# Boese0601/RC-MVSNet

Hardware: AMD Instinct MI355X
Metric: ref-scenes/sec (DTU 3-view 512x640, D=48/32/8) (higher is better)
Workload: dtype f32; 1 GPU; BASELINE configs[1]: CascadeMVSNet_eval.forward, DTU-shaped 3 views 512x640, D=(48,32,8), batch 1 per GPU, fp32, random-init seeded weights; views=3, height=512, width=640, parallelism=scene-per-gpu x1, ranks=1, procs_per_gpu=1, rccl_ranks=0

## Files before the change

rc_mvsnet_amd/_lib.py:

```python
import ast
import ctypes
import os
import re
import subprocess

_HERE = os.path.dirname(os.path.abspath(__file__))
LIB_PATH = os.path.join(_HERE, "librcmvs_hip.so")
CSRC = os.path.join(_HERE, "csrc")
HEADER = os.path.join(os.path.dirname(_HERE), "include", "rcmvs.h")

_lib = None


class RcmvsError(RuntimeError):
    pass


_CTYPES = {"int": ctypes.c_int, "float": ctypes.c_float, "double": ctypes.c_double, "long long": ctypes.c_longlong}


def _const_expr(text):
    def ev(node):
        if isinstance(node, ast.Constant) and type(node.value) is int:
            return node.value
        if isinstance(node, ast.BinOp) and isinstance(node.op, ast.LShift):
            return ev(node.left) << ev(node.right)
        raise ValueError(text)
    return ev(ast.parse(text.strip(), mode="eval").body)


def _ctype(decl, what, c_type):
    if c_type not in _CTYPES:
        raise RcmvsError(f"{HEADER}: `{decl}`: {what} type `{c_type}` is outside the ABI's types ({', '.join(_CTYPES)}, pointers)")
    return _CTYPES[c_type]


def parse_header(text):
    text = re.sub(r"/\*.*?\*/|//[^\n]*", " ", text, flags=re.S)
    signatures, restypes, constants, code = {}, {}, {}, []
    for line in text.splitlines():
        if not line.lstrip().startswith("#"):
            code.append(line)
            continue
        m = re.match(r"\s*#\s*define\s+(RCMVS_\w+)\s+(\S.*)", line)
        if m:
            try:
                value = _const_expr(m.group(2))
            except (ValueError, SyntaxError):
                raise RcmvsError(f"{HEADER}: `{line.strip()}`: not an integer expression of literals, << and parentheses") from None
            if m.group(1) in constants:
                raise RcmvsError(f"{HEADER}: {m.group(1)} is defined twice")
            constants[m.group(1)] = value
    for decl in re.sub(r'extern\s+"C"\s*\{', " ", "\n".join(code)).split(";"):
        decl = " ".join(decl.split())
        if "rcmvs_" not in decl:
            continue
        m = re.fullmatch(r"([\w\s*]+?)\s*\b(rcmvs_\w+)\s*\(([^()]*)\)", decl)
        if not m:
            raise RcmvsError(f"{HEADER}: `{decl}` is not a complete `<type> rcmvs_name(<parameters>);` declaration")
        ret, name, params = m.group(1), m.group(2), m.group(3).strip()
        if name in signatures:
            raise RcmvsError(f"{HEADER}: {name} is declared twice")
        if ret.replace("const", "").replace(" ", "") == "char*":
            restypes[name] = ctypes.c_char_p
        elif ret != "int":
            restypes[name] = _ctype(decl, "return", ret)
        argtypes = []
        for param in ([] if params == "void" else params.split(",")):
            if "*" in param:
                argtypes.append(ctypes.c_void_p)
                continue
            words = [w for w in param.split() if w != "const"]
            if len(words) < 2 or not words[-1].isidentifier():
                raise RcmvsError(f"{HEADER}: `{decl}`: parameter `{param.strip()}` is not `<type> <name>`")
            argtypes.append(_ctype(decl, "parameter", " ".join(words[:-1])))
        signatures[name] = argtypes
    return signatures, restypes, constants


def _read_header():
    try:
        with open(HEADER) as f:
            return f.read()
    except FileNotFoundError:
        raise RcmvsError(f"{HEADER} is missing: the ctypes binding is derived from the C header, which was expected there "
                         "(include/rcmvs.h next to the rc_mvsnet_amd package)") from None


SIGNATURES, _RESTYPES, CONSTANTS = parse_header(_read_header())
REQUIRED_VERSION = CONSTANTS["RCMVS_VERSION"]


def sources():
    return sorted(os.path.join(CSRC, f) for f in os.listdir(CSRC) if f.endswith(".hip"))


def build(force=False, verbose=False):
    from concurrent.futures import ThreadPoolExecutor
    srcs = sources()
    hdrs = [os.path.join(CSRC, f) for f in os.listdir(CSRC) if f.endswith(".h")] + [HEADER]
    if not force and os.path.exists(LIB_PATH) and all(os.path.getmtime(LIB_PATH) >= os.path.getmtime(d) for d in srcs + hdrs):
        return LIB_PATH
    hipcc = os.environ.get("HIPCC", "/opt/rocm/bin/hipcc")
    objdir = os.path.join(_HERE, "_obj")
    os.makedirs(objdir, exist_ok=True)
    hdr_time = max(os.path.getmtime(h) for h in hdrs)
    jobs, objs = [], []
    for src in srcs:
        obj = os.path.join(objdir, os.path.basename(src)[:-4] + ".o")
        objs.append(obj)
        if force or not os.path.exists(obj) or os.path.getmtime(obj) < max(os.path.getmtime(src), hdr_time):
            jobs.append([hipcc, "--offload-arch=gfx950", "-O3", "-std=c++17", "-fPIC", "-c", src, "-o", obj])

    def run(cmd):
        if verbose:
            print(" ".join(cmd), flush=True)
        subprocess.run(cmd, check=True)

    with ThreadPoolExecutor(max_workers=min(8, os.cpu_count() or 1)) as ex:
        list(ex.map(run, jobs))
    run([hipcc, "--offload-arch=gfx950", "-shared", "-fPIC", "-o", LIB_PATH] + objs)
    return LIB_PATH


def load():
    global _lib
    if _lib is not None:
        return _lib
    path = os.environ.get("RCMVS_LIB") or LIB_PATH
    if not os.path.exists(path):
        raise RcmvsError(f"{path} is missing: run `python -c 'import __graft_entry__ as g; g.build()'` "
                         "(hipcc --offload-arch=gfx950). There is no CPU / eager fallback.")
    lib = ctypes.CDLL(path)
    for name, argtypes in SIGNATURES.items():
        fn = getattr(lib, name)
        fn.argtypes = argtypes
        fn.restype = _RESTYPES.get(name, ctypes.c_int)
    if lib.rcmvs_version() < REQUIRED_VERSION:
        raise RcmvsError(f"librcmvs_hip.so (version {lib.rcmvs_version()}) is older than this package needs ({REQUIRED_VERSION}): rebuild it")
    _lib = lib
    return lib


def check(rc, what):
    if rc != 0:
        msg = load().rcmvs_last_error_string()
        raise RcmvsError(f"{what} failed (rc={rc}): {msg.decode() if msg else ''}")


def call(name, *args):
    rc = getattr(_lib or load(), name)(*args)
    if rc:
        check(rc, name[len("rcmvs_"):])
```

rc_mvsnet_amd/casmvsnet.py:

```python
import os

FP16_PAIR_DEFAULT = True
ONE_BY_ONE_MFMA = os.environ.get("RCMVS_1X1_MFMA", "1") != "0"
HEAD_PAIR = os.environ.get("RCMVS_HEAD_PAIR", "1") != "0"
CONV11_PROB = int(os.environ.get("RCMVS_CONV11_PROB", "1"))
CONV_TILE = os.environ.get("RCMVS_CONV_TILE", "1") != "0"
CONV_STEM = os.environ.get("RCMVS_CONV_STEM", "1") != "0"
CONV_PAIR = os.environ.get("RCMVS_CONV_PAIR", "1") != "0"
DEEP_PAIR = os.environ.get("RCMVS_DEEP_PAIR", "1") != "0"

import torch
import torch.nn as nn
import torch.nn.functional as F

from . import ops
from ._lib import RcmvsError


def _nhwc(x):
    x = x.contiguous().float()
    return ops.rgb_to_nhwc4(x) if x.shape[1] == 3 else ops.to_channels_last(x)


def _param(mod, name):
    p = mod._parameters.get(name)
    return p if p is not None else getattr(mod, name)


def _packed_of(module, make):
    w = module.conv.weight
    key = (w.data_ptr(), w._version, str(w.device))
    c = module.__dict__.get("_rcmvs_pack")
    if c is None or c[0] != key:
        c = module.__dict__["_rcmvs_pack"] = (key, make(w.detach()))
    return c[1]


def _affine_of(m):
    if getattr(m, "gn", None) is not None:
        raise RcmvsError(f"{type(m).__name__}: GroupNorm blocks are not provided (the reference builds every block with norm='batch_norm')")
    if m.bn is not None:
        return _bn_fold(m.bn)
    b = m.conv.bias
    if b is None:
        return None, None
    return torch.ones_like(b, dtype=torch.float32), b.detach().float().contiguous()


def _same2(v, n):
    return tuple(v) == (n, n)


def _conv2d_block_cl(m, t):
    conv = m.conv
    K = conv.kernel_size[0]
    st = conv.stride[0]
    if (not _same2(conv.kernel_size, K) or K not in (1, 3, 5) or not _same2(conv.padding, K // 2) or not _same2(conv.stride, st)
            or st not in (1, 2) or not _same2(conv.dilation, 1) or conv.groups != 1 or conv.padding_mode != "zeros"):
        raise RcmvsError(f"Conv2d: only square 1x1 / 3x3 / 5x5 kernels with 'same' zero padding, stride 1 or 2, no dilation or groups "
                         f"(the layers of models/modules.py) run on the HIP path; got {conv}")
    scale, shift = _affine_of(m)
    relu = bool(m.relu)
    if K == 5 or conv.in_channels == 3:
        pw = _packed_of(m, lambda w: ops.pack_conv2d_weight(w, pad_in_to=4 if w.shape[1] == 3 else None))
        return ops.conv2d(t, pw, scale, shift, stride=st, relu=relu)
    pw = _packed_of(m, lambda w: ops.pack_conv3d_weight(FeatureNet._w3(w)))
    return ops.conv3d(t.unsqueeze(1), pw, scale, shift, stride=st, relu=relu).squeeze(1)


def _deconv2d_block_cl(m, t):
    conv = m.conv
    if (not _same2(conv.kernel_size, 3) or not _same2(conv.stride, 2) or not _same2(conv.padding, 1) or not _same2(conv.output_padding, 1)
            or not _same2(conv.dilation, 1) or conv.groups != 1):
        raise RcmvsError(f"Deconv2d: only kernel 3, stride 2, padding 1, output_padding 1 (DeConv2dFuse, models/modules.py:346) runs on the "
                         f"HIP path; got {conv}")
    if m.bn is None:
        raise RcmvsError("Deconv2d: bn=False is not provided (the reference's forward returns its INPUT in that case, models/modules.py:106-110)")
    scale, shift = _bn_fold(m.bn)
    pw = _packed_of(m, lambda w: ops.pack_conv3d_weight(F.pad(w.unsqueeze(2), (0, 0, 0, 0, 1, 1)), transposed=True))
    return ops.deconv3d(t.unsqueeze(1), pw, scale, shift, relu=bool(m.relu))[:, 0]


class Conv2d(nn.Module):
    def __init__(self, in_channels, out_channels, kernel_size, stride=1, relu=True, bn=True, bn_momentum=0.1,
                 init_method="xavier", **kwargs):
        super().__init__()
        self.conv = nn.Conv2d(in_channels, out_channels, kernel_size, stride=stride, bias=(not bn), **kwargs)
        self.kernel_size = kernel_size
        self.stride = stride
        self.bn = nn.BatchNorm2d(out_channels, momentum=bn_momentum) if bn else None
        self.relu = relu

    def forward(self, x):
        if _hip_inference(self, x):
            return ops.to_channels_first(_conv2d_block_cl(self, _nhwc(x)).contiguous())
        _unsupported(self, x)


class Deconv2d(nn.Module):

    def __init__(self, in_channels, out_channels, kernel_size, stride=1, relu=True, bn=True, bn_momentum=0.1,
                 init_method="xavier", **kwargs):
        super().__init__()
        assert stride in [1, 2]
        self.out_channels = out_channels
        self.stride = stride
        self.conv = nn.ConvTranspose2d(in_channels, out_channels, kernel_size, stride=stride, bias=(not bn), **kwargs)
        self.bn = nn.BatchNorm2d(out_channels, momentum=bn_momentum) if bn else None
        self.relu = relu

    def forward(self, x):
        if _hip_inference(self, x):
            return ops.to_channels_first(_deconv2d_block_cl(self, _nhwc(x)).contiguous())
        _unsupported(self, x)


class DeConv2dFuse(nn.Module):

    def __init__(self, in_channels, out_channels, kernel_size, relu=True, bn=True, bn_momentum=0.1):
        super().__init__()
        self.deconv = Deconv2d(in_channels, out_channels, kernel_size, stride=2, padding=1, output_padding=1, bn=True, relu=relu,
                               bn_momentum=bn_momentum)
        self.conv = Conv2d(2 * out_channels, out_channels, kernel_size, stride=1, padding=1, bn=bn, relu=relu, bn_momentum=bn_momentum)

    def forward_cl(self, x_pre, x):
        up = _deconv2d_block_cl(self.deconv, x)
        if up.shape != x_pre.shape:
            raise RcmvsError(f"DeConv2dFuse: the skip map {tuple(x_pre.shape)} is not twice the size of the up-sampled one {tuple(up.shape)}")
        return _conv2d_block_cl(self.conv, torch.cat((up, x_pre), dim=-1))

    def forward(self, x_pre, x):
        if _hip_inference(self, x_pre, x):
            return ops.to_channels_first(self.forward_cl(_nhwc(x_pre), _nhwc(x)).contiguous())
        _unsupported(self, x_pre, x)


class FeatureNet(nn.Module):

    def __init__(self, base_channels, num_stage=3, stride=4, arch_mode="fpn"):
        super().__init__()
        if arch_mode not in ("unet", "fpn"):
            raise ValueError("mode must be in 'unet' or 'fpn', but get:{}".format(arch_mode))
        if num_stage not in (1, 2, 3):
            raise ValueError("num_stage must be 1, 2 or 3")
        self.arch_mode = arch_mode
        self.stride = stride
        self.base_channels = base_channels
        self.num_stage = num_stage
        b = base_channels
        self.conv0 = nn.Sequential(Conv2d(3, b, 3, 1, padding=1), Conv2d(b, b, 3, 1, padding=1))
        self.conv1 = nn.Sequential(Conv2d(b, b * 2, 5, stride=2, padding=2), Conv2d(b * 2, b * 2, 3, 1, padding=1),
                                   Conv2d(b * 2, b * 2, 3, 1, padding=1))
        self.conv2 = nn.Sequential(Conv2d(b * 2, b * 4, 5, stride=2, padding=2), Conv2d(b * 4, b * 4, 3, 1, padding=1),
                                   Conv2d(b * 4, b * 4, 3, 1, padding=1))
        self.out1 = nn.Conv2d(b * 4, b * 4, 1, bias=False)
        self.out_channels = [4 * b]
        final_chs = b * 4
        if arch_mode == "unet":
            if num_stage >= 2:
                self.deconv1 = DeConv2dFuse(b * 4, b * 2, 3)
                self.out2 = nn.Conv2d(b * 2, b * 2, 1, bias=False)
                self.out_channels.append(2 * b)
            if num_stage == 3:
                self.deconv2 = DeConv2dFuse(b * 2, b, 3)
                self.out3 = nn.Conv2d(b, b, 1, bias=False)
                self.out_channels.append(b)
        elif num_stage == 3:
            self.inner1 = nn.Conv2d(b * 2, final_chs, 1, bias=True)
            self.inner2 = nn.Conv2d(b * 1, final_chs, 1, bias=True)
            self.out2 = nn.Conv2d(final_chs, b * 2, 3, padding=1, bias=False)
            self.out3 = nn.Conv2d(final_chs, b, 3, padding=1, bias=False)
            self.out_channels += [b * 2, b]
        elif num_stage == 2:
            self.inner1 = nn.Conv2d(b * 2, final_chs, 1, bias=True)
            self.out2 = nn.Conv2d(final_chs, b, 3, padding=1, bias=False)
            self.out_channels.append(b)

    def hip_plan(self):
        sub = self._modules
        mods = [m for seq in ("conv0", "conv1", "conv2") for m in sub[seq]._modules.values()]
        tens = []
        for m in mods:
            cv, bn = m._modules["conv"], m._modules["bn"]
            bb = bn._buffers
            tens += [_param(cv, "weight"), _param(bn, "weight"), _param(bn, "bias"), bb["running_mean"], bb["running_var"], bb["num_batches_tracked"]]
        unet = self.arch_mode == "unet"
        heads = ["out1"] + (["out2", "out3"] if unet else ["inner1", "out2", "inner2", "out3"])
        extra = [t for n in heads if n in sub for t in (_param(sub[n], "weight"), getattr(sub[n], "bias", None)) if t is not None]
        key = tuple((t.data_ptr(), t._version) for t in tens + extra)
        if getattr(self, "_plan", None) is None or key != self._plan_key:
            plan = {}
            names = ["conv0.0", "conv0.1", "conv1.0", "conv1.1", "conv1.2", "conv2.0", "conv2.1", "conv2.2"]
            for n, m in zip(names, mods):
                pad_to = 4 if m.conv.in_channels == 3 else None
                w = m.conv.weight
                if tuple(w.shape) in ((8, 8, 3, 3), (16, 16, 3, 3), (32, 32, 3, 3)) and m.stride == 1:
                    w3 = w.detach().new_zeros(w.shape[0], w.shape[1], 3, 3, 3)
                    w3[:, :, 1] = w.detach()
                    plan[n] = ("mfma3d", ops.pack_conv3d_weight(w3)) + _bn_fold(m.bn)
                    continue
                if tuple(w.shape) in ((32, 16, 5, 5), (16, 8, 5, 5)) and m.stride == 2:
                    w3 = self._w3(self._w5s2(w.detach())).contiguous()
                    plan[n] = ("s2d_mfma3d", ops.pack_conv3d_weight(w3)) + _bn_fold(m.bn)
                    continue
                plan[n] = (ops.pack_conv2d_weight(w, pad_in_to=pad_to),) + _bn_fold(m.bn) + (m.stride,)
            m11, m12 = mods[3], mods[4]
            if CONV_PAIR and all(tuple(m.conv.weight.shape) == (16, 16, 3, 3) and m.stride == 1 for m in (m11, m12)):
                plan["pair1"] = (ops.pack_conv2d_pair(m11.conv.weight, m12.conv.weight),) + _bn_fold(m11.bn) + _bn_fold(m12.bn)
            m00, m01 = mods[0], mods[1]
            if CONV_STEM and tuple(m00.conv.weight.shape) == (8, 3, 3, 3) and tuple(m01.conv.weight.shape) == (8, 8, 3, 3) and m00.stride == 1 and m01.stride == 1:
                plan["stem"] = (plan["conv0.0"][0],) + _bn_fold(m00.bn) + (ops.pack_conv2d_stem(m01.conv.weight),) + _bn_fold(m01.bn)
            m10 = mods[2]
            if CONV_TILE and tuple(m10.conv.weight.shape) == (16, 8, 5, 5) and m10.stride == 2:
                plan["tile10"] = (ops.pack_conv2d_tile(self._w5s2(m10.conv.weight.detach()).contiguous()),) + _bn_fold(m10.bn)
            for n, m in (("conv2.1", mods[6]), ("conv2.2", mods[7])):
                if CONV_TILE and tuple(m.conv.weight.shape) == (32, 32, 3, 3) and m.stride == 1:
                    plan["tile:" + n] = (ops.pack_conv2d_tile(m.conv.weight),) + _bn_fold(m.bn)
            plan["out1"] = ops.pack_conv2d_weight(self.out1.weight)
            if unet:
                for n in ("out2", "out3")[:self.num_stage - 1]:
                    plan[n] = ops.pack_conv3d_weight(self._w3(getattr(self, n).weight.detach()))
            elif self.num_stage >= 2:
                plan["inner1"] = (ops.pack_conv2d_weight(self.inner1.weight), self.inner1.bias.detach().float().contiguous())
                if tuple(self.out2.weight.shape) == (16, 32, 3, 3):
                    w3 = self.out2.weight.detach().new_zeros(16, 32, 3, 3, 3)
                    w3[:, :, 1] = self.out2.weight.detach()
                    plan["out2"] = ("mfma3d", ops.pack_conv3d_weight(w3))
                    if CONV_TILE:
                        plan["out2t"] = ops.pack_conv2d_tile(self.out2.weight)
                else:
                    plan["out2"] = ops.pack_conv2d_weight(self.out2.weight)
            if self.num_stage == 3 and not unet:
                plan["inner2"] = (ops.pack_conv2d_weight(self.inner2.weight), self.inner2.bias.detach().float().contiguous())
                plan["out3"] = ops.pack_conv2d_weight(self.out3.weight)
                plan["fuse_out3"] = tuple(self.inner2.weight.shape[:2]) == (32, 8) and tuple(self.out3.weight.shape[:2]) == (8, 32)
                if plan["fuse_out3"]:
                    plan["fold_out3"] = ops.pack_fpn_folded(self.inner2.weight, self.inner2.bias, self.out3.weight)
                    if os.environ.get("RCMVS_FPN_MFMA", "1") != "0":
                        plan["fold_out3"] = ops.pack_fpn_folded_mfma(plan["fold_out3"])
            self._plan, self._plan_key = plan, key
        return self._plan

    def forward_cl(self, x, lazy=False):
        p = self.hip_plan()

        def cbr(t, n):
            if "tile:" + n in p and not ops._CONV_IMPL:
                img, sc, sh = p["tile:" + n]
                return ops.conv2d_tile(t, img, sc, sh, relu=True)
            if p[n][0] == "mfma3d":
                _, w3, sc, sh = p[n]
                return ops.conv3d(t.unsqueeze(1), w3, sc, sh, relu=True).squeeze(1)
            if p[n][0] == "s2d_mfma3d":
                if t.shape[1] % 2 or t.shape[2] % 2:
                    raise RcmvsError(f"FeatureNet: image height and width must be multiples of 4 (got a {t.shape[1]}x{t.shape[2]} map "
                                     "at the second stride-2 layer), as the reference's three-level pyramid requires")
                _, w3, sc, sh = p[n]
                if ops._CONV_IMPL:
                    return ops.conv3d(self._s2d(t).contiguous().unsqueeze(1), w3, sc, sh, relu=True).squeeze(1)
                return ops.conv2d_s2d(t, w3, sc, sh, relu=True)
            w, sc, sh, stride = p[n]
            return ops.conv2d(t, w, sc, sh, stride=stride, relu=True)

        w00 = p["conv0.0"][0] if len(p["conv0.0"]) == 4 else None
        if "stem" in p and not ops._CONV_IMPL:
            c0 = ops.conv2d_stem(x.contiguous().float(), *p["stem"])
        else:
            c0 = None
        if c0 is not None:
            pass
        elif w00 is not None and w00.ci == 4 and w00.co == 8 and w00.k == 3 and p["conv0.0"][3] == 1 and not ops._CONV_IMPL:
            w, sc, sh, _ = p["conv0.0"]
            c0 = cbr(ops.conv2d_rgb(x.contiguous().float(), w, sc, sh, relu=True), "conv0.1")
        else:
            c0 = cbr(cbr(ops.rgb_to_nhwc4(x.contiguous().float()), "conv0.0"), "conv0.1")
        if "tile10" in p and not ops._CONV_IMPL and c0.shape[1] % 2 == 0 and c0.shape[2] % 2 == 0:
            c10 = ops.conv2d_tile(c0, p["tile10"][0], p["tile10"][1], p["tile10"][2], relu=True, s2d=True)
        else:
            c10 = cbr(c0, "conv1.0")
        if "pair1" in p and not ops._CONV_IMPL:
            c1 = ops.conv2d_pair(c10, *p["pair1"])
        else:
            c1 = cbr(cbr(c10, "conv1.1"), "conv1.2")
        c2 = cbr(cbr(cbr(c1, "conv2.0"), "conv2.1"), "conv2.2")
        def out1(bound=None, t=c2):
            if tuple(self.out1.weight.shape) == (32, 32, 1, 1) and (bound is not None or ONE_BY_ONE_MFMA):
                return ops.conv1x1(t, p["out1"], ysq_absmax=bound, mfma=ONE_BY_ONE_MFMA), bound is not None
            return ops.conv2d(t, p["out1"]), False
        out = {"stage1": out1}
        plain = lambda f: (lambda bound=None: (f(), False))
        if self.arch_mode == "unet":
            one = lambda t, n: ops.conv3d(t.unsqueeze(1), p[n]).squeeze(1)
            if self.num_stage >= 2:
                intra = self.deconv1.forward_cl(c1, c2)
                out["stage2"] = plain(lambda t=intra: one(t, "out2"))
            if self.num_stage == 3:
                intra = self.deconv2.forward_cl(c0, intra)
                out["stage3"] = plain(lambda t=intra: one(t, "out3"))
            return out if lazy else {k: f()[0] for k, f in out.items()}
        if self.num_stage >= 2:
            intra = ops.conv2d(c1, p["inner1"][0], None, p["inner1"][1], up_add=c2)
            if isinstance(p["out2"], tuple):
                def out2(bound=None, t=intra):
                    keep = bound is not None and not ops._CONV_IMPL
                    if "out2t" in p and not ops._CONV_IMPL:
                        return ops.conv2d_tile(t, p["out2t"], ysq_absmax=bound), keep
                    return ops.conv3d(t.unsqueeze(1), p["out2"][1], y_absmax=bound if keep else None, y_absmax_square=keep).squeeze(1), keep
                out["stage2"] = out2
            else:
                out["stage2"] = plain(lambda t=intra: ops.conv2d(t, p["out2"]))
        if self.num_stage == 3:
            if p.get("fuse_out3") and c0.shape[1] % 2 == 0 and c0.shape[2] % 2 == 0:
                if p.get("fold_out3") is not None:
                    out["stage3"] = (lambda bound=None, a=c0, b=intra: (ops.fpn_out_folded(a, b, p["fold_out3"], ysq_absmax=bound), bound is not None))
                else:
                    out["stage3"] = plain(lambda a=c0, b=intra: ops.fpn_out_fused(a, b, p["inner2"][0], p["inner2"][1], p["out3"]))
            else:
                intra = ops.conv2d(c0, p["inner2"][0], None, p["inner2"][1], up_add=intra)
                out["stage3"] = plain(lambda t=intra: ops.conv2d(t, p["out3"]))
        return out if lazy else {k: f()[0] for k, f in out.items()}

    @staticmethod
    def _w3(w):
        p = (3 - w.shape[-1]) // 2
        return F.pad(w.unsqueeze(2), (p, p, p, p, 1, 1))

    @staticmethod
    def _w5s2(w):
        Co, Ci = w.shape[:2]
        w6 = F.pad(w, (0, 1, 0, 1))
        return w6.reshape(Co, Ci, 3, 2, 3, 2).permute(0, 3, 5, 1, 2, 4).reshape(Co, 4 * Ci, 3, 3)

    @staticmethod
    def _s2d(x):
        N, H, W, C = x.shape
        return x.reshape(N, H // 2, 2, W // 2, 2, C).permute(0, 1, 3, 2, 4, 5).reshape(N, H // 2, W // 2, 4 * C)

    def forward_train_cl(self, x, segments=1):
        from .train_ops import ConvPlainFn, conv_bn_train_w
        if self.arch_mode != "fpn":
            raise RcmvsError("FeatureNet(arch_mode='unet'): the train-mode HIP path covers the shipped 'fpn' pyramid only (the one-plane form of "
                             "its transposed convs would put the discarded plane into the batch statistics)")
        N, _, H, W = x.shape
        if H % 4 or W % 4:
            raise RcmvsError("FeatureNet (training): image height and width must be multiples of 4")
        t = F.pad(x.permute(0, 2, 3, 1), (0, 5)).contiguous()

        def cbr(t, m):
            w = m.conv.weight
            if m.stride == 2:
                t, w = self._s2d(t), self._w5s2(w)
            return conv_bn_train_w(self._w3(w), m.bn, t.unsqueeze(1), relu=True, segments=segments).squeeze(1)

        def plain(t, conv):
            return ConvPlainFn.apply(t.unsqueeze(1), self._w3(conv.weight), conv.bias).squeeze(1)

        def up2(t):
            return t.repeat_interleave(2, dim=1).repeat_interleave(2, dim=2)

        c0 = t
        for m in self.conv0: c0 = cbr(c0, m)
        c1 = c0
        for m in self.conv1: c1 = cbr(c1, m)
        c2 = c1
        for m in self.conv2: c2 = cbr(c2, m)
        out = {"stage1": plain(c2, self.out1)}
        intra = c2
        if self.num_stage >= 2:
            intra = up2(intra) + plain(c1, self.inner1)
            out["stage2"] = plain(intra, self.out2)
        if self.num_stage == 3:
            intra = up2(intra) + plain(c0, self.inner2)
            out["stage3"] = plain(intra, self.out3)
        return out

    def forward(self, x):
        if _hip_inference(self, x):
            return {k: ops.to_channels_first(v) for k, v in self.forward_cl(x).items()}
        if _hip_training(self, x):
            return {k: v.permute(0, 3, 1, 2) for k, v in self.forward_train_cl(x).items()}
        _unsupported(self, x)


class Conv3d(nn.Module):
    def __init__(self, in_channels, out_channels, kernel_size=3, stride=1, relu=True, bn=True, bn_momentum=0.1, **kwargs):
        super().__init__()
        assert stride in [1, 2]
        self.out_channels = out_channels
        self.kernel_size = kernel_size
        self.stride = stride
        self.conv = nn.Conv3d(in_channels, out_channels, kernel_size, stride=stride, bias=(not bn), **kwargs)
        self.bn = nn.BatchNorm3d(out_channels, momentum=bn_momentum)
        self.gn = None
        self.relu = relu

    def forward(self, x):
        return _block3d(self, x)


class Deconv3d(nn.Module):
    def __init__(self, in_channels, out_channels, kernel_size=3, stride=1, relu=True, bn=True, bn_momentum=0.1, **kwargs):
        super().__init__()
        assert stride in [1, 2]
        self.out_channels = out_channels
        self.stride = stride
        self.conv = nn.ConvTranspose3d(in_channels, out_channels, kernel_size, stride=stride, bias=(not bn), **kwargs)
        self.bn = nn.BatchNorm3d(out_channels, momentum=bn_momentum)
        self.gn = None
        self.relu = relu

    def forward(self, x):
        return _block3d(self, x)


def _block3d(m, x):
    conv = m.conv
    transposed = isinstance(conv, nn.ConvTranspose3d)
    ok = (_same3(conv.kernel_size, 3) and _same3(conv.padding, 1) and _same3(conv.dilation, 1) and conv.groups == 1
          and (_same3(conv.stride, 2) and _same3(conv.output_padding, 1) if transposed
               else conv.stride[0] in (1, 2) and _same3(conv.stride, conv.stride[0]) and conv.padding_mode == "zeros"))
    if not ok:
        raise RcmvsError(f"{type(m).__name__}: only kernel 3, padding 1 (transposed: stride 2, output_padding 1) -- the layers of "
                         f"CostRegNet, models/modules.py:473-487 -- run on the HIP path; got {conv}")
    if _hip_inference(m, x):
        scale, shift = _affine_of(m)
        pw = _packed_of(m, lambda w: ops.pack_conv3d_weight(w, transposed=transposed))
        t = ops.to_channels_last(x.contiguous().float())
        y = ops.deconv3d(t, pw, scale, shift, relu=bool(m.relu)) if transposed else ops.conv3d(t, pw, scale, shift, stride=conv.stride[0], relu=bool(m.relu))
        return ops.to_channels_first(y)
    if _hip_training(m, x):
        if m.bn is None or conv.bias is not None:
            raise RcmvsError(f"{type(m).__name__}: the train-mode HIP path is conv -> BatchNorm (batch statistics) -> [ReLU] without a bias")
        from .train_ops import conv_bn_relu_train
        return conv_bn_relu_train(m, x.float().permute(0, 2, 3, 4, 1).contiguous()).permute(0, 4, 1, 2, 3)
    _unsupported(m, x)


def _same3(v, n):
    return tuple(v) == (n, n, n)


def _bn_fold(bn):
    scale = bn.weight.detach() / torch.sqrt(bn.running_var + bn.eps)
    shift = bn.bias.detach() - bn.running_mean * scale
    return scale.float().contiguous(), shift.float().contiguous()


class CostRegNet(nn.Module):

    _LAYERS = ("conv0", "conv1", "conv2", "conv3", "conv4", "conv5", "conv6", "conv7", "conv9", "conv11")
    BOUND_ROWS = 11

    def __init__(self, in_channels, base_channels):
        super().__init__()
        b = base_channels
        self.conv0 = Conv3d(in_channels, b, padding=1)
        self.conv1 = Conv3d(b, b * 2, stride=2, padding=1)
        self.conv2 = Conv3d(b * 2, b * 2, padding=1)
        self.conv3 = Conv3d(b * 2, b * 4, stride=2, padding=1)
        self.conv4 = Conv3d(b * 4, b * 4, padding=1)
        self.conv5 = Conv3d(b * 4, b * 8, stride=2, padding=1)
        self.conv6 = Conv3d(b * 8, b * 8, padding=1)
        self.conv7 = Deconv3d(b * 8, b * 4, stride=2, padding=1, output_padding=1)
        self.conv9 = Deconv3d(b * 4, b * 2, stride=2, padding=1, output_padding=1)
        self.conv11 = Deconv3d(b * 2, b * 1, stride=2, padding=1, output_padding=1)
        self.prob = nn.Conv3d(b, 1, 3, stride=1, padding=1, bias=False)
        self._plan = None
        self._plan_key = None

    def _tensors(self):
        ts = []
        mods = self._modules
        for n in self._LAYERS:
            m = mods[n]._modules
            cv, bn = m["conv"], m["bn"]
            bb = bn._buffers
            ts += [_param(cv, "weight"), _param(bn, "weight"), _param(bn, "bias"), bb["running_mean"], bb["running_var"], bb["num_batches_tracked"]]
        ts.append(_param(mods["prob"], "weight"))
        return ts

    def hip_plan(self):
        key = tuple((t.data_ptr(), t._version) for t in self._tensors())
        if self._plan is None or key != self._plan_key:
            plan = {}
            for n in self._LAYERS:
                m = getattr(self, n)
                w = ops.pack_conv3d_weight(m.conv.weight, transposed=isinstance(m, Deconv3d))
                s, b = _bn_fold(m.bn)
                plan[n] = (w, s, b)
            plan["prob"] = ops.pack_conv3d_weight(self.prob.weight)
            plan["conv11_coef"] = self._conv11_bound_coef(plan["conv11"][1], plan["conv11"][2])
            self._plan, self._plan_key = plan, key
        return self._plan

    def _conv11_bound_coef(self, scale, shift):
        w = self.conv11.conv.weight.detach().float().abs().sum(0)
        taps = ([1], [0, 2])
        l1 = None
        for pd in range(2):
            for ph in range(2):
                for pw in range(2):
                    v = w[:, taps[pd]][:, :, taps[ph]][:, :, :, taps[pw]].sum((1, 2, 3))
                    l1 = v if l1 is None else torch.maximum(l1, v)
        c1 = (scale.abs() * l1).max() * (1.0 + 2.0 ** -10)
        c2 = shift.abs().max() * (1.0 + 2.0 ** -10)
        return torch.stack((c1, c2)).float().contiguous()

    def features_cl(self, x, x_absmax=None, plan=None, logits=False, planes=None):
        B, D, h, w, _ = x.shape
        if D % 8 or h % 8 or w % 8:
            raise RcmvsError(f"CostRegNet: volume {D}x{h}x{w} must be divisible by 8 in every axis "
                             "(three stride-2 levels with skip connections, models/modules.py:492-499)")
        p = self.hip_plan() if plan is None else plan
        if logits and (x_absmax is None or B != 1):
            raise RcmvsError("CostRegNet.features_cl(logits=True): the fused conv11 + prob pass is the fp16-pair form of a B = 1 scene")
        if x_absmax is None:
            conv0 = ops.conv3d(x, *p["conv0"], relu=True)
            conv2 = ops.conv3d(ops.conv3d(conv0, *p["conv1"], stride=2, relu=True), *p["conv2"], relu=True)
            conv4 = ops.conv3d(ops.conv3d(conv2, *p["conv3"], stride=2, relu=True), *p["conv4"], relu=True)
            t = ops.conv3d(ops.conv3d(conv4, *p["conv5"], stride=2, relu=True), *p["conv6"], relu=True)
            t = ops.deconv3d(t, *p["conv7"], residual=conv4, relu=True)
            t = ops.deconv3d(t, *p["conv9"], residual=conv2, relu=True)
            return ops.deconv3d(t, *p["conv11"], residual=conv0, relu=True)
        b = [x_absmax[i] for i in range(1, self.BOUND_ROWS)]
        x_absmax = x_absmax[0]
        conv0 = ops.conv3d(x, *p["conv0"], relu=True, x_absmax=x_absmax, y_absmax=b[0])
        conv1 = ops.conv3d(conv0, *p["conv1"], stride=2, relu=True, x_absmax=b[0], y_absmax=b[1])
        conv2 = ops.conv3d(conv1, *p["conv2"], relu=True, x_absmax=b[1], y_absmax=b[2])
        conv3 = ops.conv3d(conv2, *p["conv3"], stride=2, relu=True, x_absmax=b[2], y_absmax=b[3])
        if DEEP_PAIR:
            conv4 = ops.conv3d(conv3, *p["conv4"], relu=True, x_absmax=b[3], y_absmax=b[6])
            t = ops.conv3d(conv4, *p["conv5"], stride=2, relu=True, x_absmax=b[6], y_absmax=b[7])
            t = ops.conv3d(t, *p["conv6"], relu=True, x_absmax=b[7], y_absmax=b[8])
            t = ops.deconv3d(t, *p["conv7"], residual=conv4, relu=True, x_absmax=b[8], y_absmax=b[5])
        else:
            conv4 = ops.conv3d(conv3, *p["conv4"], relu=True, x_absmax=b[3])
            t = ops.conv3d(ops.conv3d(conv4, *p["conv5"], stride=2, relu=True), *p["conv6"], relu=True)
            t = ops.deconv3d(t, *p["conv7"], residual=conv4, relu=True, y_absmax=b[5])
        t = ops.deconv3d(t, *p["conv9"], residual=conv2, relu=True, x_absmax=b[5], y_absmax=b[4])
        if logits:
            return ops.conv11_prob(t, b[4], p["conv11"][0], p["conv11"][1], p["conv11"][2], conv0, b[0], p["conv11_coef"], p["prob"], planes=planes)
        return ops.deconv3d(t, *p["conv11"], residual=conv0, relu=True, x_absmax=b[4], y_absmax=b[9])

    def features_cl_train(self, x):
        from .train_ops import conv_bn_relu_train as blk
        B, D, h, w, _ = x.shape
        if D % 8 or h % 8 or w % 8:
            raise RcmvsError(f"CostRegNet: volume {D}x{h}x{w} must be divisible by 8 in every axis")
        conv0 = blk(self.conv0, x)
        conv2 = blk(self.conv2, blk(self.conv1, conv0))
        conv4 = blk(self.conv4, blk(self.conv3, conv2))
        t = blk(self.conv6, blk(self.conv5, conv4))
        t = blk(self.conv7, t, residual=conv4)
        t = blk(self.conv9, t, residual=conv2)
        return blk(self.conv11, t, residual=conv0)

    def forward(self, x):
        if _hip_inference(self, x):
            feat = self.features_cl(ops.to_channels_last(x.contiguous().float()))
            logits = ops.conv3d(feat, self.hip_plan()["prob"])
            return ops.to_channels_first(logits)
        _unsupported(self, x)


def _hip_inference(module, *tensors):
    return (not module.training) and (not torch.is_grad_enabled()) and all(t.is_cuda for t in tensors)


def _hip_training(module, *tensors):
    return module.training and all(t.is_cuda for t in tensors)


def _unsupported(module, *tensors):
    name = type(module).__name__
    if not all(t.is_cuda for t in tensors):
        raise RcmvsError(f"{name}: the HIP path needs its tensors on the GPU (there is no CPU / eager fallback)")
    raise RcmvsError(f"{name}: eval-mode forward with autograd enabled is not provided -- wrap inference in torch.no_grad(), "
                     "or put the module in train() mode for the differentiable HIP path")


def _holder_only(module):
    raise RcmvsError(f"{type(module).__name__} is a parameter holder: its conv / bn children are executed by the enclosing "
                     "network's HIP plan (Rendering_Consistency_Net.forward and its volume / MLP chains)")


class DepthNet(nn.Module):

    def __init__(self, train_variant):
        super().__init__()
        self.train_variant = train_variant

    def forward(self, features, proj_matrices, depth_values, num_depth, cost_regularization, imgs=None, pad=0, prob_volume_init=None):
        if pad != 0 or prob_volume_init is not None:
            raise RcmvsError("DepthNet: pad and prob_volume_init are not provided (no caller of the reference passes them)")
        V = len(features)
        B, C, h, w = features[0].shape
        D = int(num_depth)
        if proj_matrices.shape[1] != V:
            raise RcmvsError("DepthNet: different number of images and projection matrices")
        if tuple(depth_values.shape) != (B, D, h, w):
            raise RcmvsError(f"DepthNet: depth_values {tuple(depth_values.shape)} is not (B, num_depth, h, w) = {(B, D, h, w)}")
        dv = depth_values.float()
        d0 = dv[:, 0]
        delta = (dv[:, 1] - d0) if D > 1 else torch.zeros_like(d0)
        k = torch.arange(D, device=dv.device, dtype=torch.float32).view(1, D, 1, 1)
        if float((dv - (d0.unsqueeze(1) + k * delta.unsqueeze(1))).abs().max()) > 1e-5 * float(dv.abs().max()):
            raise RcmvsError("DepthNet: depth_values must be uniformly spaced along the depth axis at every pixel (d_0 + k * delta)")
        planes = torch.stack((d0, delta), dim=-1).contiguous()
        with torch.no_grad():
            rot, trans = ops.compose_homography(proj_matrices.contiguous().float())
            small_cl = None
            if self.train_variant:
                if imgs is None:
                    raise RcmvsError("DepthNet (train variant): imgs (B,V,3,H,W) are needed for volume_feature_no_ref")
                small_cl = ops.resize_rgb_cl(imgs.float().reshape(B * V, *imgs.shape[2:]).contiguous(), (h, w)).view(B, V, h, w, 3)
        if _hip_inference(self, *features, depth_values):
            f_cl = torch.stack([ops.to_channels_last(f.contiguous().float()) for f in features], dim=1)
            var = ops.warp_variance(f_cl, rot, trans, planes, D)
            x8 = cost_regularization.features_cl(var)
            depth, conf = ops.depth_head(x8, cost_regularization.hip_plan()["prob"], planes)
            out = {"depth": depth, "photometric_confidence": conf}
            if self.train_variant:
                out["volume_feature_no_ref"] = ops.warp_noref(f_cl, small_cl, rot, trans, planes, D, square_first=True)
            return out
        if _hip_training(self, *features, depth_values):
            from . import train_ops
            f_cl = torch.stack([f.float().permute(0, 2, 3, 1) for f in features], dim=1).contiguous()
            res = ops.WarpVarianceFn.apply(f_cl, rot, trans, planes, D, small_cl)
            var, noref = res if self.train_variant else (res, None)
            x8 = cost_regularization.features_cl_train(var)
            depth, conf = train_ops.ProbDepthHeadFn.apply(x8, cost_regularization.prob.weight, planes)
            out = {"depth": depth, "photometric_confidence": conf}
            if self.train_variant:
                out["volume_feature_no_ref"] = noref
            return out
        _unsupported(self, *features, depth_values)


class _CascadeBase(nn.Module):
    TRAIN_VARIANT = False

    def __init__(self, refine=False, ndepths=[48, 32, 8], depth_interals_ratio=[4, 2, 1], share_cr=False,
                 grad_method="detach", arch_mode="fpn", cr_base_chs=[8, 8, 8]):
        super().__init__()
        if refine:
            raise NotImplementedError("refine=True: the reference's RefineNet is not runnable (models/modules.py:511 calls F.cat)")
        self.refine = refine
        self.share_cr = share_cr
        self.ndepths = ndepths
        self.depth_interals_ratio = depth_interals_ratio
        self.grad_method = grad_method
        self.arch_mode = arch_mode
        self.cr_base_chs = cr_base_chs
        self.num_stage = len(ndepths)
        assert len(ndepths) == len(depth_interals_ratio)
        self.stage_infos = {"stage1": {"scale": 4.0}, "stage2": {"scale": 2.0}, "stage3": {"scale": 1.0}}
        self.feature = FeatureNet(base_channels=8, stride=4, num_stage=self.num_stage, arch_mode=self.arch_mode)
        if self.share_cr:
            self.cost_regularization = CostRegNet(in_channels=self.feature.out_channels, base_channels=8)
        else:
            self.cost_regularization = nn.ModuleList([CostRegNet(in_channels=self.feature.out_channels[i],
                                                                 base_channels=self.cr_base_chs[i])
                                                      for i in range(self.num_stage)])
        self.DepthNet = DepthNet(self.TRAIN_VARIANT)

    def _cr(self, s):
        return self.cost_regularization if self.share_cr else self.cost_regularization[s]

    def _forward_hip(self, imgs, proj_matrices, depth_values, features=None, homographies=None):
        B, V, _, H, W = imgs.shape
        imgs = imgs.float()
        depth_values = depth_values.contiguous().float()
        feats_cl = None
        if features is None:
            feats_cl = self.feature.forward_cl(imgs.reshape(B * V, 3, H, W), lazy=True)
        outputs = {}
        depth = None
        bounds = None
        need_fill = False
        pair = getattr(self, "fp16_pair", None)
        if pair is None:
            pair = FP16_PAIR_DEFAULT if os.environ.get("RCMVS_FP16_PAIR") is None else os.environ["RCMVS_FP16_PAIR"] == "1"
        if pair and B == 1:
            bounds = getattr(self, "_pair_bounds", None)
            if getattr(self, "_is_replica", False):
                bounds = torch.zeros(self.num_stage, CostRegNet.BOUND_ROWS, ops.ABSMAX_FLOATS, device=imgs.device, dtype=torch.float32)
            elif bounds is None or bounds.device != imgs.device:
                bounds = self._pair_bounds = torch.zeros(self.num_stage, CostRegNet.BOUND_ROWS, ops.ABSMAX_FLOATS, device=imgs.device, dtype=torch.float32)
            else:
                need_fill = True
        if homographies is None:
            if self.num_stage <= 4:
                rots, transs = ops.compose_homography_stages([proj_matrices["stage{}".format(k + 1)].contiguous().float() for k in range(self.num_stage)],
                                                             zero=bounds if need_fill else None)
                need_fill = False
            else:
                rt = [ops.compose_homography(proj_matrices["stage{}".format(k + 1)].contiguous().float()) for k in range(self.num_stage)]
                rots, transs = [r for r, _ in rt], [t for _, t in rt]
        if need_fill:
            bounds.zero_()
        for s in range(self.num_stage):
            key = "stage{}".format(s + 1)
            scale = int(self.stage_infos[key]["scale"])
            D = self.ndepths[s]
            bound_kept = False
            if feats_cl is not None:
                fk, bound_kept = feats_cl[key](bounds[s][0] if bounds is not None else None)
                h, w, C = fk.shape[1:]
                f_cl = fk.view(B, V, h, w, C)
            else:
                C, h, w = features[key].shape[1:]
                f_cl = ops.to_channels_last(features[key].contiguous()).view(B, V, h, w, C)
            if homographies is not None:
                rot, trans = homographies[key]
            else:
                rot, trans = rots[s], transs[s]
            planes = ops.hypothesis_planes(depth, depth_values, (H, W), scale, D, self.depth_interals_ratio[s])
            var = ops.warp_variance(f_cl, rot, trans, planes, D, uniform_planes=depth is None)
            cr = self._cr(s)
            vmax = None
            if bounds is not None:
                vmax = bounds[s]
                if not bound_kept:
                    ops.absmax(f_cl, square=True, out=vmax[0])
            plan = cr.hip_plan()
            if vmax is not None and HEAD_PAIR and (CONV11_PROB == 2 or (CONV11_PROB == 1 and D == 8)):
                depth, conf = cr.features_cl(var, vmax, plan, logits=True, planes=planes)
            else:
                x8 = cr.features_cl(var, vmax, plan)
                depth, conf = ops.depth_head(x8, plan["prob"], planes, x_absmax=vmax[CostRegNet.BOUND_ROWS - 1] if vmax is not None and HEAD_PAIR else None)
            out = {"depth": depth, "photometric_confidence": conf}
            if self.TRAIN_VARIANT:
                small_cl = ops.resize_rgb_cl(imgs.reshape(B * V, 3, H, W).contiguous(), (h, w)).view(B, V, h, w, 3)
                out["volume_feature_no_ref"] = ops.warp_noref(f_cl, small_cl, rot, trans, planes, D, square_first=True)
            outputs[key] = out
            outputs.update(out)
        return outputs

    def _forward_train_hip(self, imgs, proj_matrices, depth_values):
        from . import train_ops
        B, V, _, H, W = imgs.shape
        imgs = imgs.float()
        depth_values = depth_values.contiguous().float()
        fv = self.feature.forward_train_cl(imgs.transpose(0, 1).reshape(V * B, 3, H, W), segments=V)
        features = [{k: f[v * B:(v + 1) * B] for k, f in fv.items()} for v in range(V)]
        outputs = {}
        depth = None
        for s in range(self.num_stage):
            key = "stage{}".format(s + 1)
            scale = int(self.stage_infos[key]["scale"])
            D = self.ndepths[s]
            f_cl = torch.stack([f[key] for f in features], dim=1).contiguous()
            h, w = f_cl.shape[2:4]
            with torch.no_grad():
                rot, trans = ops.compose_homography(proj_matrices[key].contiguous().float())
                prev = depth.detach() if depth is not None else None
                planes = ops.hypothesis_planes(prev, depth_values, (H, W), scale, D, self.depth_interals_ratio[s])
                small_cl = None
                if self.TRAIN_VARIANT:
                    small_cl = ops.resize_rgb_cl(imgs.reshape(B * V, 3, H, W).contiguous(), (h, w)).view(B, V, h, w, 3)
            res = ops.WarpVarianceFn.apply(f_cl, rot, trans, planes, D, small_cl)
            var, noref = res if self.TRAIN_VARIANT else (res, None)
            cr = self._cr(s)
            x8 = cr.features_cl_train(var)
            prev_live = depth
            depth, conf = train_ops.ProbDepthHeadFn.apply(x8, cr.prob.weight, planes)
            if prev_live is not None and self.grad_method != "detach":
                up = F.interpolate(prev_live.unsqueeze(1), [H, W], mode="bilinear", align_corners=False)
                base = F.interpolate(up, [h, w], mode="bilinear", align_corners=False).squeeze(1)
                depth = depth + (base - base.detach())
            out = {"depth": depth, "photometric_confidence": conf}
            if self.TRAIN_VARIANT:
                out["volume_feature_no_ref"] = noref
            outputs[key] = out
            outputs.update(out)
        return outputs

    def _run(self, imgs, proj_matrices, depth_values):
        if _hip_inference(self, imgs, depth_values):
            return self._forward_hip(imgs, proj_matrices, depth_values)
        if _hip_training(self, imgs, depth_values):
            return self._forward_train_hip(imgs, proj_matrices, depth_values)
        _unsupported(self, imgs, depth_values)


class CascadeMVSNet_eval(_CascadeBase):
    TRAIN_VARIANT = False

    def forward(self, imgs, proj_matrices, depth_values):
        return self._run(imgs, proj_matrices, depth_values)


class CascadeMVSNet(_CascadeBase):
    TRAIN_VARIANT = True

    def forward(self, imgs, proj_matrices, depth_values):
        outputs = self._run(imgs, proj_matrices, depth_values)
        return outputs, outputs["stage1"]["volume_feature_no_ref"]
```

rc_mvsnet_amd/csrc/conv2d.hip:

```cpp
#include "common.h"
#include "x3_pieces.h"

namespace rcmvs {

typedef float f4v __attribute__((ext_vector_type(4)));

constexpr int C2_CK = 8;
constexpr int C2_STRIDE = C2_CK + 4;

template <int CI, int CO, int K, int S, int TH, int TW, int PPT, int UKY, int UKX, bool RGB3 = false>
__global__ __launch_bounds__(256) void conv2d_lds_kernel(
    const float* __restrict__ x, const float* __restrict__ wp, const float* __restrict__ scale,
    const float* __restrict__ shift, const float* __restrict__ up, float* __restrict__ y,
    int H, int W, int Ho, int Wo, int tiles_w, int relu) {
    static_assert(!RGB3 || CI == 4, "planar RGB input feeds the 4-channel first layer");
    static_assert(TH * TW == 256, "tile must have 256 threads");
    constexpr int PAD = K / 2;
    constexpr int HH = (TH * PPT - 1) * S + K, HW = (TW - 1) * S + K;
    constexpr int CKW = (CI < C2_CK ? CI : C2_CK) * CO;
    extern __shared__ __attribute__((aligned(16))) float tile[];
    const int n = blockIdx.y;
    const unsigned t2 = xcd_remap(blockIdx.x, gridDim.x);
    const int tw = t2 % tiles_w, th = t2 / tiles_w;
    const int oy0 = th * TH * PPT, ox0 = tw * TW;
    const int lx = threadIdx.x % TW, ly = threadIdx.x / TW;
    const int ox = ox0 + lx;
    const float* xb = x + (long long)n * H * W * (RGB3 ? 3 : CI);
    const int iy0 = oy0 * S - PAD, ix0 = ox0 * S - PAD;

    static_assert(CO % 2 == 0, "output channels are accumulated in pairs");
    typedef float f2v __attribute__((ext_vector_type(2)));
    f2v acc2[PPT][CO / 2];
#pragma unroll
    for (int p = 0; p < PPT; ++p)
#pragma unroll
        for (int c = 0; c < CO / 2; ++c) acc2[p][c] = (f2v){0.0f, 0.0f};

    for (int c0 = 0; c0 < CI; c0 += C2_CK) {
        const int ck = (CI - c0 < C2_CK) ? (CI - c0) : C2_CK;
        const int q = ck >> 2;
        if (c0 > 0) __syncthreads();
        for (int e = threadIdx.x; e < HH * HW * q; e += 256) {
            const int v = e / q, c4 = e - v * q;
            const int hx = v % HW, hy = v / HW;
            const int iy = iy0 + hy, ix = ix0 + hx;
            float4 val = make_float4(0.f, 0.f, 0.f, 0.f);
            if (iy >= 0 && iy < H && ix >= 0 && ix < W) {
                if constexpr (RGB3) {
                    const long long pix = (long long)iy * W + ix, hw = (long long)H * W;
                    val = make_float4(xb[pix], xb[hw + pix], xb[2 * hw + pix], 0.0f);
                } else {
                    val = *reinterpret_cast<const float4*>(xb + ((long long)iy * W + ix) * CI + c0 + c4 * 4);
                }
            }
            *reinterpret_cast<float4*>(tile + v * C2_STRIDE + c4 * 4) = val;
        }
        __syncthreads();
#pragma unroll UKY
        for (int ky = 0; ky < K; ++ky) {
#pragma unroll UKX
            for (int kx = 0; kx < K; ++kx) {
                const float* wt = wp + ((long long)(ky * K + kx) * CI + c0) * CO;
#pragma unroll
                for (int c4 = 0; c4 < C2_CK / 4; ++c4) {
                    if (c4 * 4 < ck) {
                        f4v xv[PPT];
#pragma unroll
                        for (int p = 0; p < PPT; ++p)
                            xv[p] = *reinterpret_cast<const f4v*>(tile + (((ly + p * TH) * S + ky) * HW + (lx * S + kx)) * C2_STRIDE + c4 * 4);
                        if constexpr (PPT > 1 || CO <= 8) {
#pragma unroll
                            for (int j = 0; j < 4; ++j) {
#pragma unroll
                                for (int co = 0; co < CO; co += 2) {
                                    if constexpr (K > 1) {
                                        const f2v wv = (f2v){wt[(c4 * 4 + j) * CO + co], wt[(c4 * 4 + j) * CO + co + 1]};
#pragma unroll
                                        for (int p = 0; p < PPT; ++p) acc2[p][co / 2] = __builtin_elementwise_fma((f2v){xv[p][j], xv[p][j]}, wv, acc2[p][co / 2]);
                                    } else {
                                        const float w0 = wt[(c4 * 4 + j) * CO + co], w1 = wt[(c4 * 4 + j) * CO + co + 1];
#pragma unroll
                                        for (int p = 0; p < PPT; ++p) {
                                            acc2[p][co / 2].x = fmaf(xv[p][j], w0, acc2[p][co / 2].x);
                                            acc2[p][co / 2].y = fmaf(xv[p][j], w1, acc2[p][co / 2].y);
                                        }
                                    }
                                }
                            }
                        } else {
#pragma unroll
                            for (int co = 0; co < CO; co += 2) {
#pragma unroll
                                for (int j = 0; j < 4; ++j)
                                    acc2[0][co / 2] = __builtin_elementwise_fma((f2v){xv[0][j], xv[0][j]}, (f2v){wt[(c4 * 4 + j) * CO + co], wt[(c4 * 4 + j) * CO + co + 1]}, acc2[0][co / 2]);
                            }
                        }
                    }
                }
            }
        }
    }
    float acc[PPT][CO];
#pragma unroll
    for (int p = 0; p < PPT; ++p)
#pragma unroll
        for (int c = 0; c < CO / 2; ++c) { acc[p][2 * c] = acc2[p][c].x; acc[p][2 * c + 1] = acc2[p][c].y; }
#pragma unroll
    for (int p = 0; p < PPT; ++p) {
        const int oy = oy0 + ly + p * TH;
        if (!(oy < Ho && ox < Wo)) continue;
        const long long op = ((long long)n * Ho + oy) * Wo + ox;
        float* yp = y + op * CO;
        const float* upp = up ? up + (((long long)n * (Ho / 2) + oy / 2) * (Wo / 2) + ox / 2) * CO : nullptr;
        if (scale) {
#pragma unroll
            for (int co = 0; co < CO; ++co) acc[p][co] = acc[p][co] * scale[co];
        }
        if (shift) {
#pragma unroll
            for (int co = 0; co < CO; ++co) acc[p][co] = acc[p][co] + shift[co];
        }
        if (upp) {
#pragma unroll
            for (int co = 0; co < CO; co += 4) {
                const f4v u4 = *reinterpret_cast<const f4v*>(upp + co);
                acc[p][co] = u4.x + acc[p][co]; acc[p][co + 1] = u4.y + acc[p][co + 1];
                acc[p][co + 2] = u4.z + acc[p][co + 2]; acc[p][co + 3] = u4.w + acc[p][co + 3];
            }
        }
        if (relu) {
#pragma unroll
            for (int co = 0; co < CO; ++co) acc[p][co] = fmaxf(acc[p][co], 0.0f);
        }
#pragma unroll
        for (int co = 0; co < CO; co += 4)
            *reinterpret_cast<float4*>(yp + co) = make_float4(acc[p][co], acc[p][co + 1], acc[p][co + 2], acc[p][co + 3]);
    }
}

template <int CI, int CO, bool TRS>
__global__ __launch_bounds__(256) void conv1x1_kernel(
    const float* __restrict__ x, const float* __restrict__ wp, const float* __restrict__ scale, const float* __restrict__ shift,
    const float* __restrict__ up, float* __restrict__ y, float* __restrict__ ysq, long long npix, int H, int W, int relu) {
    __shared__ float red[4];
    __shared__ __attribute__((aligned(16))) float tr[TRS ? 256 * (CO + 4) : 4];
    const long long p = (long long)blockIdx.x * 256 + threadIdx.x;
    const bool live = p < npix;
    float acc[CO];
#pragma unroll
    for (int co = 0; co < CO; ++co) acc[co] = 0.0f;
    float m = 0.0f;
    if (live) {
        f4v xv[CI / 4];
#pragma unroll
        for (int c = 0; c < CI / 4; ++c) xv[c] = *reinterpret_cast<const f4v*>(x + p * CI + c * 4);
#pragma unroll 2
        for (int c = 0; c < CI / 4; ++c) {
#pragma unroll
            for (int j = 0; j < 4; ++j) {
                const float* wt = wp + (c * 4 + j) * CO;
#pragma unroll
                for (int co = 0; co < CO; ++co) acc[co] = fmaf(xv[c][j], wt[co], acc[co]);
            }
        }
        if (scale) {
#pragma unroll
            for (int co = 0; co < CO; ++co) acc[co] = acc[co] * scale[co];
        }
        if (shift) {
#pragma unroll
            for (int co = 0; co < CO; ++co) acc[co] = acc[co] + shift[co];
        }
        if (up) {
            const long long hw = (long long)H * W;
            const long long n = p / hw;
            const int r = (int)(p - n * hw), oy = r / W, ox = r - oy * W;
            const float* upp = up + ((n * (H / 2) + oy / 2) * (W / 2) + ox / 2) * CO;
#pragma unroll
            for (int co = 0; co < CO; co += 4) {
                const f4v u4 = *reinterpret_cast<const f4v*>(upp + co);
                acc[co] = u4.x + acc[co]; acc[co + 1] = u4.y + acc[co + 1]; acc[co + 2] = u4.z + acc[co + 2]; acc[co + 3] = u4.w + acc[co + 3];
            }
        }
        if (relu) {
#pragma unroll
            for (int co = 0; co < CO; ++co) acc[co] = fmaxf(acc[co], 0.0f);
        }
        if (ysq) {
#pragma unroll
            for (int co = 0; co < CO; ++co) m = fmaxf(m, fabsf(acc[co]));
        }
    }
    if constexpr (!TRS) {
        if (live) {
            float* yp = y + p * CO;
#pragma unroll
            for (int co = 0; co < CO; co += 4) *reinterpret_cast<float4*>(yp + co) = make_float4(acc[co], acc[co + 1], acc[co + 2], acc[co + 3]);
        }
    } else {
        constexpr int STR = CO + 4;
        float* tw = tr + (threadIdx.x >> 6) * 64 * STR;
        const int lane = threadIdx.x & 63;
#pragma unroll
        for (int co = 0; co < CO; co += 4) *reinterpret_cast<f4v*>(tw + lane * STR + co) = (f4v){acc[co], acc[co + 1], acc[co + 2], acc[co + 3]};
        __builtin_amdgcn_wave_barrier();
        const long long wbase = (long long)blockIdx.x * 256 + (threadIdx.x & ~63);
#pragma unroll
        for (int i = 0; i < CO / 4; ++i) {
            const int e = i * 64 + lane, px = e / (CO / 4), q = e % (CO / 4);
            const f4v v = *reinterpret_cast<const f4v*>(tw + px * STR + q * 4);
            if (wbase + px < npix) *reinterpret_cast<f4v*>(y + (wbase + px) * CO + q * 4) = v;
        }
    }
    if (ysq) {
#pragma unroll
        for (int k = 32; k > 0; k >>= 1) m = fmaxf(m, __shfl_xor(m, k));
        if ((threadIdx.x & 63) == 0) red[threadIdx.x >> 6] = m;
        __syncthreads();
        if (threadIdx.x == 0) {
            m = fmaxf(fmaxf(red[0], red[1]), fmaxf(red[2], red[3]));
            atomicMax(reinterpret_cast<unsigned int*>(ysq) + (blockIdx.x & 63) * 16, __float_as_uint(m * m));
        }
    }
}

template <int CI, int CO>
static int conv1x1_launch_t(const float* x, const float* wp, const float* scale, const float* shift, const float* up, float* y, float* ysq,
                            int N, int H, int W, int relu, hipStream_t st) {
    const long long npix = (long long)N * H * W;
    if (npix >= 131072)
        hipLaunchKernelGGL((conv1x1_kernel<CI, CO, true>), dim3((unsigned)((npix + 255) / 256)), dim3(256), 0, st, x, wp, scale, shift, up, y, ysq, npix, H, W, relu);
    else
        hipLaunchKernelGGL((conv1x1_kernel<CI, CO, false>), dim3((unsigned)((npix + 255) / 256)), dim3(256), 0, st, x, wp, scale, shift, up, y, ysq, npix, H, W, relu);
    return launch_status("conv1x1");
}

__global__ void pack_weight2d_kernel(const float* __restrict__ w, float* __restrict__ packed, int Co, int Ci, int Cip, int KK) {
    int t = blockIdx.x * blockDim.x + threadIdx.x;
    if (t >= KK * Cip * Co) return;
    int co = t % Co, ci = (t / Co) % Cip, tap = t / (Co * Cip);
    packed[t] = (ci < Ci) ? w[((long long)co * Ci + ci) * KK + tap] : 0.0f;
}

__global__ __launch_bounds__(256) void rgb_to_nhwc4_kernel(const float* __restrict__ x, float* __restrict__ y, long long HW) {
    const int n = blockIdx.y;
    long long p = (long long)blockIdx.x * blockDim.x + threadIdx.x;
    if (p >= HW) return;
    const float* xb = x + (long long)n * 3 * HW;
    *reinterpret_cast<float4*>(y + ((long long)n * HW + p) * 4) = make_float4(xb[p], xb[HW + p], xb[2 * HW + p], 0.0f);
}

template <int CI, int CO, int K, int S, int TH, int TW, int PPT, int UKY, int UKX, bool RGB3 = false>
static int conv2d_launch_t(const float* x, const float* wp, const float* scale, const float* shift, const float* up, float* y,
                           int N, int H, int W, int relu, hipStream_t st) {
    constexpr int PAD = K / 2;
    const int Ho = (H + 2 * PAD - K) / S + 1, Wo = (W + 2 * PAD - K) / S + 1;
    const int tiles_w = (Wo + TW - 1) / TW, tiles_h = (Ho + TH * PPT - 1) / (TH * PPT);
    constexpr int HH = (TH * PPT - 1) * S + K, HW = (TW - 1) * S + K;
    const size_t lds = (size_t)HH * HW * C2_STRIDE * sizeof(float);
    hipLaunchKernelGGL((conv2d_lds_kernel<CI, CO, K, S, TH, TW, PPT, UKY, UKX, RGB3>), dim3(tiles_w * tiles_h, N), dim3(256), lds, st, x, wp, scale,
                       shift, up, y, H, W, Ho, Wo, tiles_w, relu);
    return launch_status("conv2d");
}

template <int CI>
__global__ __launch_bounds__(256) void conv1x1_mfma_kernel(
    const float* __restrict__ x, const float* __restrict__ wp, const float* __restrict__ scale, const float* __restrict__ shift,
    const float* __restrict__ up, float* __restrict__ y, float* __restrict__ ysq, long long npix, int H, int W, int relu) {
    constexpr int CO = 32;
    constexpr int KL = CI / 4;
    static_assert(CI == 32 || CI == 16, "one k-step: Ci = 32 or 16");
    typedef short s16x4 __attribute__((ext_vector_type(4)));
    typedef unsigned int frag_t __attribute__((ext_vector_type(KL / 2)));
    __shared__ float red[4];
    const int lane = threadIdx.x & 63, wave = threadIdx.x >> 6;
    const int n = lane & 15, kq = lane >> 4;
    frag_t A[2][3];
#pragma unroll
    for (int mt = 0; mt < 2; ++mt) {
        unsigned hb[KL], mb[KL], lb[KL];
#pragma unroll
        for (int i = 0; i < KL; ++i) {
            const float v = wp[(kq * KL + i) * CO + mt * 16 + n];
            hb[i] = __float_as_uint(v) & 0xffff0000u;
            const float r1 = v - __uint_as_float(hb[i]);
            mb[i] = __float_as_uint(r1) & 0xffff0000u;
            const float r2 = r1 - __uint_as_float(mb[i]);
            lb[i] = __float_as_uint(r2) & 0xffff0000u;
        }
#pragma unroll
        for (int j = 0; j < KL / 2; ++j) {
            A[mt][0][j] = (hb[2 * j] >> 16) | hb[2 * j + 1];
            A[mt][1][j] = (mb[2 * j] >> 16) | mb[2 * j + 1];
            A[mt][2][j] = (lb[2 * j] >> 16) | lb[2 * j + 1];
        }
    }
    auto mfma = [](frag_t a, frag_t b, x3_f32x4 c) -> x3_f32x4 {
        if constexpr (KL == 8) return x3_mfma<3>(a, b, c);
        else return __builtin_amdgcn_mfma_f32_16x16x16bf16_1k(__builtin_bit_cast(s16x4, a), __builtin_bit_cast(s16x4, b), c, 0, 0, 0);
    };
    const long long ntiles = (npix + 15) / 16, stride = (long long)gridDim.x * 4;
    x3_f32x4 xq[KL / 4];
    auto fetch = [&](long long tile) {
        const long long p = tile * 16 + n;
        const bool in = tile < ntiles && p < npix;
#pragma unroll
        for (int c = 0; c < KL / 4; ++c) xq[c] = in ? *reinterpret_cast<const x3_f32x4*>(x + p * CI + kq * KL + c * 4) : (x3_f32x4){0.f, 0.f, 0.f, 0.f};
    };
    float vmax = 0.0f;
    long long tile = (long long)blockIdx.x * 4 + wave;
    fetch(tile);
    const long long hw = (long long)H * W;
    for (; tile < ntiles; tile += stride) {
        frag_t bq[3];
        {
            x3_u32x2 h0, m0, l0;
            x3_split4(xq[0], h0, m0, l0);
            if constexpr (KL == 8) {
                x3_u32x2 h1, m1, l1;
                x3_split4(xq[KL / 4 - 1], h1, m1, l1);
                bq[0] = (frag_t){h0.x, h0.y, h1.x, h1.y}; bq[1] = (frag_t){m0.x, m0.y, m1.x, m1.y}; bq[2] = (frag_t){l0.x, l0.y, l1.x, l1.y};
            } else { bq[0] = (frag_t){h0.x, h0.y}; bq[1] = (frag_t){m0.x, m0.y}; bq[2] = (frag_t){l0.x, l0.y}; }
        }
        fetch(tile + stride);
        const long long p = tile * 16 + n;
        const bool live = p < npix;
        long long upo = 0;
        if (up && live) {
            const long long b = p / hw;
            const int r = (int)(p - b * hw), oy = r / W, ox = r - oy * W;
            upo = ((b * (H / 2) + oy / 2) * (W / 2) + ox / 2) * CO;
        }
#pragma unroll
        for (int mt = 0; mt < 2; ++mt) {
            x3_f32x4 acc[3] = {(x3_f32x4){0.f, 0.f, 0.f, 0.f}, (x3_f32x4){0.f, 0.f, 0.f, 0.f}, (x3_f32x4){0.f, 0.f, 0.f, 0.f}};
            acc[2] = mfma(A[mt][0], bq[2], acc[2]);
            acc[1] = mfma(A[mt][0], bq[1], acc[1]);
            acc[0] = mfma(A[mt][0], bq[0], acc[0]);
            acc[2] = mfma(A[mt][1], bq[1], acc[2]);
            acc[1] = mfma(A[mt][1], bq[0], acc[1]);
            acc[2] = mfma(A[mt][2], bq[0], acc[2]);
            const int co = mt * 16 + kq * 4;
            x3_f32x4 v = acc[0] + (acc[1] + acc[2]);
            if (scale) v = v * *reinterpret_cast<const x3_f32x4*>(scale + co);
            if (shift) v = v + *reinterpret_cast<const x3_f32x4*>(shift + co);
            if (live) {
                if (up) v = *reinterpret_cast<const x3_f32x4*>(up + upo + co) + v;
                if (relu) v = __builtin_elementwise_max(v, (x3_f32x4){0.f, 0.f, 0.f, 0.f});
                *reinterpret_cast<x3_f32x4*>(y + p * CO + co) = v;
                vmax = x3_absmax4(vmax, v);
            }
        }
    }
    if (ysq) {
#pragma unroll
        for (int k = 32; k > 0; k >>= 1) vmax = fmaxf(vmax, __shfl_xor(vmax, k));
        if (lane == 0) red[wave] = vmax;
        __syncthreads();
        if (threadIdx.x == 0) {
            const float m = fmaxf(fmaxf(red[0], red[1]), fmaxf(red[2], red[3]));
            atomicMax(reinterpret_cast<unsigned int*>(ysq) + (blockIdx.x & 63) * 16, __float_as_uint(m * m));
        }
    }
}

template <int CI>
static int conv1x1_mfma_launch_t(const float* x, const float* wp, const float* scale, const float* shift, const float* up, float* y, float* ysq,
                                 int N, int H, int W, int relu, hipStream_t st) {
    const long long npix = (long long)N * H * W, ntiles = (npix + 15) / 16;
    const long long blocks = (ntiles + 3) / 4 < 2048 ? (ntiles + 3) / 4 : 2048;
    hipLaunchKernelGGL(conv1x1_mfma_kernel<CI>, dim3((unsigned)blocks), dim3(256), 0, st, x, wp, scale, shift, up, y, ysq, npix, H, W, relu);
    return launch_status("conv1x1_mfma");
}

}

using namespace rcmvs;

extern "C" {

int rcmvs_rgb_to_nhwc4(const float* x, float* y, int N, int H, int W, void* stream) {
    RCMVS_REQUIRE(x && y && N > 0 && H > 0 && W > 0, "rgb_to_nhwc4: bad arguments");
    long long HW = (long long)H * W;
    hipLaunchKernelGGL(rgb_to_nhwc4_kernel, dim3((unsigned)cdiv(HW, 256), N), dim3(256), 0, as_stream(stream), x, y, HW);
    return launch_status("rgb_to_nhwc4");
}

int rcmvs_pack_conv2d_weight(const float* w, float* packed, int Co, int Ci, int Cip, int K, void* stream) {
    RCMVS_REQUIRE(w && packed && Co > 0 && Ci > 0 && Cip >= Ci && K > 0, "pack_conv2d_weight: bad arguments");
    int n = K * K * Cip * Co;
    hipLaunchKernelGGL(pack_weight2d_kernel, dim3((n + 255) / 256), dim3(256), 0, as_stream(stream), w, packed, Co, Ci, Cip, K * K);
    return launch_status("pack_conv2d_weight");
}

int rcmvs_conv1x1_fwd(const float* x, const float* w_packed, const float* scale, const float* shift, const float* up_add,
                      float* y, float* ysq_absmax, int N, int H, int W, int Ci, int Co, int relu, void* stream) {
    RCMVS_REQUIRE(x && w_packed && y, "conv1x1_fwd: null pointer");
    RCMVS_REQUIRE(N > 0 && H > 0 && W > 0, "conv1x1_fwd: bad sizes");
    RCMVS_REQUIRE(!up_add || (H % 2 == 0 && W % 2 == 0), "conv1x1_fwd: the up-add merge needs even H and W (got %d x %d)", H, W);
    hipStream_t st = as_stream(stream);
    if (Ci == 16 && Co == 32) return conv1x1_launch_t<16, 32>(x, w_packed, scale, shift, up_add, y, ysq_absmax, N, H, W, relu, st);
    if (Ci == 32 && Co == 32) return conv1x1_launch_t<32, 32>(x, w_packed, scale, shift, up_add, y, ysq_absmax, N, H, W, relu, st);
    if (Ci == 8 && Co == 32) return conv1x1_launch_t<8, 32>(x, w_packed, scale, shift, up_add, y, ysq_absmax, N, H, W, relu, st);
    return fail(-1, "conv1x1_fwd: unsupported layer Ci=%d Co=%d (16 -> 32, 32 -> 32, 8 -> 32)", Ci, Co);
}

int rcmvs_conv1x1_mfma_fwd(const float* x, const float* w_packed, const float* scale, const float* shift, const float* up_add,
                           float* y, float* ysq_absmax, int N, int H, int W, int Ci, int Co, int relu, void* stream) {
    RCMVS_REQUIRE(x && w_packed && y, "conv1x1_mfma_fwd: null pointer");
    RCMVS_REQUIRE(N > 0 && H > 0 && W > 0, "conv1x1_mfma_fwd: bad sizes");
    RCMVS_REQUIRE(!up_add || (H % 2 == 0 && W % 2 == 0), "conv1x1_mfma_fwd: the up-add merge needs even H and W (got %d x %d)", H, W);
    hipStream_t st = as_stream(stream);
    if (Ci == 16 && Co == 32) return conv1x1_mfma_launch_t<16>(x, w_packed, scale, shift, up_add, y, ysq_absmax, N, H, W, relu, st);
    if (Ci == 32 && Co == 32) return conv1x1_mfma_launch_t<32>(x, w_packed, scale, shift, up_add, y, ysq_absmax, N, H, W, relu, st);
    return fail(-1, "conv1x1_mfma_fwd: unsupported layer Ci=%d Co=%d (16 -> 32, 32 -> 32)", Ci, Co);
}

int rcmvs_conv2d_fwd(const float* x, const float* w_packed, const float* scale, const float* shift, const float* up_add,
                     float* y, int N, int H, int W, int Ci, int Co, int K, int stride, int relu, void* stream) {
    RCMVS_REQUIRE(x && w_packed && y, "conv2d_fwd: null pointer");
    RCMVS_REQUIRE(N > 0 && H > 0 && W > 0, "conv2d_fwd: bad sizes");
    hipStream_t st = as_stream(stream);
    if (K == 1 && stride == 1 && Co == 32 && (Ci == 8 || Ci == 16 || Ci == 32) && (!up_add || (H % 2 == 0 && W % 2 == 0)))
        return rcmvs_conv1x1_fwd(x, w_packed, scale, shift, up_add, y, nullptr, N, H, W, Ci, Co, relu, stream);
    if (Ci == 3 && Co == 8 && K == 3 && stride == 1)
        return conv2d_launch_t<4, 8, 3, 1, 16, 16, 1, 1, 3, true>(x, w_packed, scale, shift, up_add, y, N, H, W, relu, st);
#define RCMVS_C2(CI, CO, KK, SS, TH, TW, PPT, UY, UX)                                                             \
    if (Ci == CI && Co == CO && K == KK && stride == SS)                                                          \
        return conv2d_launch_t<CI, CO, KK, SS, TH, TW, PPT, UY, UX>(x, w_packed, scale, shift, up_add, y, N, H, W, relu, st);
    RCMVS_C2(4, 8, 3, 1, 16, 16, 1, 1, 3)       RCMVS_C2(8, 8, 3, 1, 16, 16, 1, 1, 1)
    RCMVS_C2(8, 16, 5, 2, 8, 32, 1, 1, 1)       RCMVS_C2(16, 16, 3, 1, 16, 16, 2, 1, 1)
    RCMVS_C2(16, 32, 5, 2, 8, 32, 1, 5, 5)      RCMVS_C2(32, 32, 3, 1, 16, 16, 1, 3, 3)
    RCMVS_C2(32, 32, 1, 1, 16, 16, 1, 1, 1)     RCMVS_C2(16, 32, 1, 1, 16, 16, 2, 1, 1)
    RCMVS_C2(32, 16, 3, 1, 16, 16, 1, 3, 3)     RCMVS_C2(8, 32, 1, 1, 16, 16, 2, 1, 1)
    RCMVS_C2(32, 8, 3, 1, 16, 16, 1, 1, 1)
#undef RCMVS_C2
    return fail(-1, "conv2d_fwd: unsupported layer Ci=%d Co=%d K=%d stride=%d", Ci, Co, K, stride);
}

}
```

rc_mvsnet_amd/csrc/depth_head.hip:

```cpp
#include "common.h"

namespace rcmvs {

int conv3d_lds_launch(const float* x, const float* wp, const float* scale, const float* shift, const float* res, float* y,
                      int B, int D, int H, int W, int Ci, int Co, int relu, hipStream_t st, int lds_cfg);
bool prob_head_fused_supported(int D, int H, int W);
bool prob_pair_supported(int D, int H, int W);
int prob_pair_launch(const float* x, const float* wimg, const float* xmax, float* y, const float* planes, float* depth, float* conf,
                     int B, int D, int H, int W, bool fuse, int zc_force, hipStream_t st);
long long prob_pair_blob_offset();
int prob_head_fused_launch(const float* x, const float* wp, const float* planes, float* depth, float* conf, float* prob,
                           int B, int D, int H, int W, hipStream_t st);

template <int LP, bool KEEP = true>
__global__ __launch_bounds__(256) void softmax_regress_kernel(float* __restrict__ prob, const float* __restrict__ planes,
                                                               float* __restrict__ depth, float* __restrict__ conf, int D, long long hw) {
    constexpr int MAXK = 16;
    const int b = blockIdx.y;
    const int j = threadIdx.x % LP;
    const long long p = ((long long)blockIdx.x * blockDim.x + threadIdx.x) / LP;
    const bool live = p < hw;
    float* col = prob + (long long)b * D * hw + (live ? p : 0);
    float v[MAXK];
    float mx = -INFINITY;
#pragma unroll
    for (int i = 0; i < MAXK; ++i) {
        const int k = j + i * LP;
        v[i] = (k < D) ? col[(long long)k * hw] : -INFINITY;
        mx = fmaxf(mx, v[i]);
    }
#pragma unroll
    for (int m = 1; m < LP; m <<= 1) mx = fmaxf(mx, __shfl_xor(mx, m));
    float sum = 0.0f;
#pragma unroll
    for (int i = 0; i < MAXK; ++i) {
        v[i] = (j + i * LP < D) ? expf(v[i] - mx) : 0.0f;
        sum += v[i];
    }
#pragma unroll
    for (int m = 1; m < LP; m <<= 1) sum += __shfl_xor(sum, m);
    const float2 pl = reinterpret_cast<const float2*>(planes)[(long long)b * hw + (live ? p : 0)];
    float dsum = 0.0f, isum = 0.0f;
#pragma unroll
    for (int i = 0; i < MAXK; ++i) {
        const int k = j + i * LP;
        v[i] = v[i] / sum;
        if (k < D) {
            if (KEEP && live) col[(long long)k * hw] = v[i];
            dsum = fmaf(v[i], fmaf((float)k, pl.y, pl.x), dsum);
            isum = fmaf(v[i], (float)k, isum);
        }
    }
#pragma unroll
    for (int m = 1; m < LP; m <<= 1) { dsum += __shfl_xor(dsum, m); isum += __shfl_xor(isum, m); }
    int idx = (int)isum;
    idx = idx < 0 ? 0 : (idx > D - 1 ? D - 1 : idx);
    float c = 0.0f;
#pragma unroll
    for (int i = 0; i < MAXK; ++i) {
        const int k = j + i * LP;
        if (k < D && k >= idx - 1 && k <= idx + 2) c += v[i];
    }
#pragma unroll
    for (int m = 1; m < LP; m <<= 1) c += __shfl_xor(c, m);
    if (live && j == 0) {
        depth[(long long)b * hw + p] = dsum;
        conf[(long long)b * hw + p] = c;
    }
}

}

using namespace rcmvs;

static int depth_head_fwd(const float* x, const float* xmax, const float* w_prob, const float* planes, float* depth, float* conf, float* prob,
                          int B, int D, int h, int w, int impl, void* stream) {
    RCMVS_REQUIRE(x && w_prob && planes && depth && conf, "depth_head_fwd: null pointer");
    RCMVS_REQUIRE(B > 0 && D > 0 && h > 0 && w > 0, "depth_head_fwd: bad sizes");
    RCMVS_REQUIRE(D <= 64, "depth_head_fwd: at most 64 depth hypotheses per stage (got %d)", D);
    hipStream_t st = as_stream(stream);
    const int zc_force = (impl >> 8) & 0xff;
    const bool pair = xmax && !(impl & 4) && prob_pair_supported(D, h, w);
    int rc;
    if (pair && D == 8 && !(impl & 1))
        return prob_pair_launch(x, w_prob + prob_pair_blob_offset(), xmax, prob, planes, depth, conf, B, D, h, w, true, 0, st);
    if (!pair && !(impl & 1) && prob_head_fused_supported(D, h, w)) return prob_head_fused_launch(x, w_prob, planes, depth, conf, prob, B, D, h, w, st);
    RCMVS_REQUIRE(prob, "depth_head_fwd: prob is required for D = %d (it doubles as the logit scratch; only the D = 8 form runs without)", D);
    if (pair) rc = prob_pair_launch(x, w_prob + prob_pair_blob_offset(), xmax, prob, nullptr, nullptr, nullptr, B, D, h, w, false, zc_force, st);
    else rc = conv3d_lds_launch(x, w_prob, nullptr, nullptr, nullptr, prob, B, D, h, w, 8, 1, 0, st, ((impl & 2) ? 16 : 0) | (zc_force << 8));
    if (rc) return rc;
    const long long hw = (long long)h * w;
    const bool keep = !(impl & 8);
#define RCMVS_SOFTMAX(LP) do { if (keep) hipLaunchKernelGGL((softmax_regress_kernel<LP, true>), dim3((unsigned)cdiv(hw * LP, 256), B), dim3(256), 0, st, prob, planes, depth, conf, D, hw); \
                               else hipLaunchKernelGGL((softmax_regress_kernel<LP, false>), dim3((unsigned)cdiv(hw * LP, 256), B), dim3(256), 0, st, prob, planes, depth, conf, D, hw); } while (0)
    if (D <= 16) RCMVS_SOFTMAX(1);
    else if (D <= 32) RCMVS_SOFTMAX(2);
    else RCMVS_SOFTMAX(4);
#undef RCMVS_SOFTMAX
    return launch_status("depth_head_fwd");
}

extern "C" int rcmvs_softmax_head_fwd(float* prob, const float* planes, float* depth, float* conf, int B, int D, int h, int w, int keep, void* stream) {
    RCMVS_REQUIRE(prob && planes && depth && conf, "softmax_head_fwd: null pointer");
    RCMVS_REQUIRE(B > 0 && D > 0 && h > 0 && w > 0, "softmax_head_fwd: bad sizes");
    RCMVS_REQUIRE(D <= 64, "softmax_head_fwd: at most 64 depth hypotheses per stage (got %d)", D);
    hipStream_t st = as_stream(stream);
    const long long hw = (long long)h * w;
#define RCMVS_SOFTMAX(LP) do { if (keep) hipLaunchKernelGGL((softmax_regress_kernel<LP, true>), dim3((unsigned)cdiv(hw * LP, 256), B), dim3(256), 0, st, prob, planes, depth, conf, D, hw); \
                               else hipLaunchKernelGGL((softmax_regress_kernel<LP, false>), dim3((unsigned)cdiv(hw * LP, 256), B), dim3(256), 0, st, prob, planes, depth, conf, D, hw); } while (0)
    if (D <= 16) RCMVS_SOFTMAX(1);
    else if (D <= 32) RCMVS_SOFTMAX(2);
    else RCMVS_SOFTMAX(4);
#undef RCMVS_SOFTMAX
    return launch_status("softmax_head_fwd");
}

extern "C" int rcmvs_depth_head_fwd(const float* x, const float* w_prob, const float* planes, float* depth, float* conf, float* prob,
                                    int B, int D, int h, int w, void* stream) {
    return depth_head_fwd(x, nullptr, w_prob, planes, depth, conf, prob, B, D, h, w, 0, stream);
}
extern "C" int rcmvs_depth_head_scaled_fwd(const float* x, const float* x_absmax, const float* w_prob, const float* planes, float* depth, float* conf,
                                           float* prob, int B, int D, int h, int w, int impl, void* stream) {
    return depth_head_fwd(x, x_absmax, w_prob, planes, depth, conf, prob, B, D, h, w, impl, stream);
}
```

rc_mvsnet_amd/csrc/geometry.hip:

```cpp
#include "common.h"

namespace rcmvs {

char* err_buf() {
    static thread_local char buf[512] = {0};
    return buf;
}

int fail(int code, const char* fmt, ...) {
    va_list ap;
    va_start(ap, fmt);
    vsnprintf(err_buf(), 512, fmt, ap);
    va_end(ap);
    return code;
}

template <bool TO_LAST>
__global__ __launch_bounds__(256) void layout_kernel(const float* __restrict__ src, float* __restrict__ dst,
                                                      int C, long long S) {
    const int Q = C >> 2;
    const int n = blockIdx.y;
    long long t = (long long)blockIdx.x * blockDim.x + threadIdx.x;
    long long sblk = t / (64LL * Q);
    int r = (int)(t % (64LL * Q));
    int q = r / 64;
    long long s = sblk * 64 + (r % 64);
    if (s >= S) return;
    const float* pl = (TO_LAST ? src : dst) + (long long)n * C * S;
    if (TO_LAST) {
        float4 v;
        v.x = pl[(4LL * q + 0) * S + s];
        v.y = pl[(4LL * q + 1) * S + s];
        v.z = pl[(4LL * q + 2) * S + s];
        v.w = pl[(4LL * q + 3) * S + s];
        *reinterpret_cast<float4*>(dst + ((long long)n * S + s) * C + 4 * q) = v;
    } else {
        float4 v = *reinterpret_cast<const float4*>(src + ((long long)n * S + s) * C + 4 * q);
        float* o = dst + (long long)n * C * S;
        o[(4LL * q + 0) * S + s] = v.x;
        o[(4LL * q + 1) * S + s] = v.y;
        o[(4LL * q + 2) * S + s] = v.z;
        o[(4LL * q + 3) * S + s] = v.w;
    }
}

template <bool TO_LAST>
__global__ __launch_bounds__(256) void layout_scalar_kernel(const float* __restrict__ src, float* __restrict__ dst,
                                                             int C, long long S) {
    const int n = blockIdx.y;
    long long t = (long long)blockIdx.x * blockDim.x + threadIdx.x;
    if (t >= S * C) return;
    long long s = t / C;
    int c = (int)(t % C);
    long long planar = ((long long)n * C + c) * S + s, last = ((long long)n * S + s) * C + c;
    if (TO_LAST) dst[last] = src[planar]; else dst[planar] = src[last];
}

template <bool TO_LAST>
static int layout_launch(const float* src, float* dst, int N, int C, long long S, void* stream) {
    RCMVS_REQUIRE(src && dst && N > 0 && C > 0 && S > 0, "layout: bad arguments N=%d C=%d S=%lld", N, C, S);
    if (C % 4 == 0) {
        long long threads = cdiv(S, 64) * 64 * (C / 4);
        dim3 grid((unsigned)cdiv(threads, 256), N);
        hipLaunchKernelGGL(layout_kernel<TO_LAST>, grid, dim3(256), 0, as_stream(stream), src, dst, C, S);
    } else {
        dim3 grid((unsigned)cdiv(S * C, 256), N);
        hipLaunchKernelGGL(layout_scalar_kernel<TO_LAST>, grid, dim3(256), 0, as_stream(stream), src, dst, C, S);
    }
    return launch_status("layout");
}

__device__ static void fold_intrinsics(const float* p, double A[4][4]) {
    for (int i = 0; i < 3; ++i)
        for (int j = 0; j < 4; ++j) {
            double s = 0.0;
            for (int k = 0; k < 3; ++k) s += (double)p[16 + i * 4 + k] * (double)p[k * 4 + j];
            A[i][j] = s;
        }
    for (int j = 0; j < 4; ++j) A[3][j] = (double)p[12 + j];
}

struct ProjPtrs { const float* p[4]; };
__global__ void compose_homography_kernel(ProjPtrs pp, float* __restrict__ rot,
                                          float* __restrict__ trans, int B, int V, float* __restrict__ zero, int zero_n) {
    for (int i = (blockIdx.y * gridDim.x + blockIdx.x) * blockDim.x + threadIdx.x; i < zero_n; i += gridDim.x * gridDim.y * blockDim.x) zero[i] = 0.0f;
    int t = blockIdx.x * blockDim.x + threadIdx.x;
    if (t >= B * (V - 1)) return;
    const float* proj = pp.p[blockIdx.y];
    rot += (long long)blockIdx.y * B * (V - 1) * 9;
    trans += (long long)blockIdx.y * B * (V - 1) * 3;
    int b = t / (V - 1), v = 1 + t % (V - 1);
    double R[4][4], S[4][4], inv[4][4];
    fold_intrinsics(proj + ((long long)b * V + 0) * 32, R);
    fold_intrinsics(proj + ((long long)b * V + v) * 32, S);
    for (int i = 0; i < 4; ++i)
        for (int j = 0; j < 4; ++j) inv[i][j] = (i == j) ? 1.0 : 0.0;
    for (int c = 0; c < 4; ++c) {
        int piv = c;
        double best = fabs(R[c][c]);
        for (int r = c + 1; r < 4; ++r)
            if (fabs(R[r][c]) > best) { best = fabs(R[r][c]); piv = r; }
        if (piv != c)
            for (int j = 0; j < 4; ++j) {
                double t0 = R[c][j]; R[c][j] = R[piv][j]; R[piv][j] = t0;
                double t1 = inv[c][j]; inv[c][j] = inv[piv][j]; inv[piv][j] = t1;
            }
        double d = 1.0 / R[c][c];
        for (int j = 0; j < 4; ++j) { R[c][j] *= d; inv[c][j] *= d; }
        for (int r = 0; r < 4; ++r) {
            if (r == c) continue;
            double f = R[r][c];
            for (int j = 0; j < 4; ++j) { R[r][j] -= f * R[c][j]; inv[r][j] -= f * inv[c][j]; }
        }
    }
    float* ro = rot + (long long)t * 9;
    float* tr = trans + (long long)t * 3;
    for (int i = 0; i < 3; ++i) {
        for (int j = 0; j < 4; ++j) {
            double s = 0.0;
            for (int k = 0; k < 4; ++k) s += S[i][k] * inv[k][j];
            if (j < 3) ro[i * 3 + j] = (float)s; else tr[i] = (float)s;
        }
    }
}

__device__ static inline float ld_agent(const float* p) {
#if defined(__AMDGCN__)
    return __hip_atomic_load(p, __ATOMIC_RELAXED, __HIP_MEMORY_SCOPE_AGENT);
#else
    return *p;
#endif
}

__device__ static inline float bilinear_up(const float* __restrict__ p, int hp, int wp, float sh, float sw, int Y, int X) {
#pragma clang fp contract(off)
    float sy = sh * ((float)Y + 0.5f) - 0.5f;
    float sx = sw * ((float)X + 0.5f) - 0.5f;
    sy = sy < 0.f ? 0.f : sy;
    sx = sx < 0.f ? 0.f : sx;
    int y0 = (int)sy, x0 = (int)sx;
    y0 = y0 > hp - 1 ? hp - 1 : y0;
    x0 = x0 > wp - 1 ? wp - 1 : x0;
    int y1 = y0 + 1 > hp - 1 ? hp - 1 : y0 + 1;
    int x1 = x0 + 1 > wp - 1 ? wp - 1 : x0 + 1;
    float ly1 = sy - (float)y0, lx1 = sx - (float)x0;
    float ly0 = 1.0f - ly1, lx0 = 1.0f - lx1;
    float top = lx0 * ld_agent(p + y0 * wp + x0) + lx1 * ld_agent(p + y0 * wp + x1);
    float bot = lx0 * ld_agent(p + y1 * wp + x0) + lx1 * ld_agent(p + y1 * wp + x1);
    return ly0 * top + ly1 * bot;
}

__global__ __launch_bounds__(256) void planes_kernel(const float* __restrict__ prev, const float* __restrict__ dv,
                                                      float* __restrict__ planes, int hp, int wp, int H, int W,
                                                      int scale, int D, float ratio, int ND) {
#pragma clang fp contract(off)
    const int h = H / scale, w = W / scale;
    const int b = blockIdx.y;
    int t = blockIdx.x * blockDim.x + threadIdx.x;
    if (t >= h * w) return;
    int y = t / w, x = t % w;
    float d0, delta;
    if (prev == nullptr) {
        float lo = dv[(long long)b * ND], hi = dv[(long long)b * ND + ND - 1];
        d0 = lo;
        delta = (hi - lo) / (float)(D - 1);
    } else {
        double itv = ((double)dv[ND - 1] - (double)dv[0]) / (double)ND;
        float half = (float)((double)D / 2.0 * ((double)ratio * itv));
        const float* p = prev + (long long)b * hp * wp;
        float sh = (float)hp / (float)H, sw = (float)wp / (float)W;
        float fd = (float)(D - 1);
        if (scale == 1) {
            float c = bilinear_up(p, hp, wp, sh, sw, y, x);
            float cmin = c - half, cmax = c + half;
            d0 = cmin;
            delta = (cmax - cmin) / fd;
        } else {
            int Y0 = y * scale + scale / 2 - 1, X0 = x * scale + scale / 2 - 1;
            float mn[2][2], it[2][2];
            for (int j = 0; j < 2; ++j)
                for (int i = 0; i < 2; ++i) {
                    float c = bilinear_up(p, hp, wp, sh, sw, Y0 + j, X0 + i);
                    float cmin = c - half, cmax = c + half;
                    mn[j][i] = cmin;
                    it[j][i] = (cmax - cmin) / fd;
                }
            d0 = 0.5f * (0.5f * mn[0][0] + 0.5f * mn[0][1]) + 0.5f * (0.5f * mn[1][0] + 0.5f * mn[1][1]);
            delta = 0.5f * (0.5f * it[0][0] + 0.5f * it[0][1]) + 0.5f * (0.5f * it[1][0] + 0.5f * it[1][1]);
        }
    }
    float2 o = make_float2(d0, delta);
    reinterpret_cast<float2*>(planes)[(long long)b * h * w + t] = o;
}

}

using namespace rcmvs;

extern "C" {

int rcmvs_version(void) { return RCMVS_VERSION; }
const char* rcmvs_last_error_string(void) { return err_buf(); }

int rcmvs_nchw_to_nhwc(const float* src, float* dst, int N, int C, long long S, void* stream) {
    return layout_launch<true>(src, dst, N, C, S, stream);
}
int rcmvs_nhwc_to_nchw(const float* src, float* dst, int N, int C, long long S, void* stream) {
    return layout_launch<false>(src, dst, N, C, S, stream);
}

int rcmvs_compose_homography(const float* proj, float* rot, float* trans, int B, int V, void* stream) {
    RCMVS_REQUIRE(proj && rot && trans, "compose_homography: null pointer");
    RCMVS_REQUIRE(B > 0 && V >= 2 && V - 1 <= RCMVS_MAX_SRC_VIEWS, "compose_homography: B=%d V=%d", B, V);
    const int n = B * (V - 1);
    ProjPtrs pp{{proj, nullptr, nullptr, nullptr}};
    hipLaunchKernelGGL(compose_homography_kernel, dim3((n + 63) / 64), dim3(64), 0, as_stream(stream), pp, rot, trans, B, V, (float*)nullptr, 0);
    return launch_status("compose_homography");
}

int rcmvs_compose_homography_stages(const float* proj0, const float* proj1, const float* proj2, const float* proj3, int nstage,
                                    float* rot, float* trans, int B, int V, float* zero, long long zero_n, void* stream) {
    RCMVS_REQUIRE(zero_n >= 0 && zero_n < (1LL << 24) && (zero || zero_n == 0), "compose_homography_stages: bad side buffer (%lld floats)", zero_n);
    RCMVS_REQUIRE(rot && trans && nstage >= 1 && nstage <= 4, "compose_homography_stages: bad arguments (1..4 stages)");
    RCMVS_REQUIRE(B > 0 && V >= 2 && V - 1 <= RCMVS_MAX_SRC_VIEWS, "compose_homography_stages: B=%d V=%d", B, V);
    ProjPtrs pp{{proj0, proj1, proj2, proj3}};
    for (int s = 0; s < nstage; ++s) RCMVS_REQUIRE(pp.p[s], "compose_homography_stages: stage %d has no projection tensor", s);
    const int n = B * (V - 1);
    hipLaunchKernelGGL(compose_homography_kernel, dim3((n + 63) / 64, nstage), dim3(zero_n ? 256 : 64), 0, as_stream(stream), pp, rot, trans, B, V, zero, (int)zero_n);
    return launch_status("compose_homography_stages");
}

int rcmvs_hypothesis_planes(const float* prev_depth, const float* depth_values, float* planes,
                            int B, int hp, int wp, int H, int W, int scale,
                            int D, float ratio, int ND, void* stream) {
    RCMVS_REQUIRE(depth_values && planes, "hypothesis_planes: null pointer");
    RCMVS_REQUIRE(B > 0 && H > 0 && W > 0 && D >= 2 && ND >= 2, "hypothesis_planes: bad sizes");
    RCMVS_REQUIRE(scale == 1 || scale == 2 || scale == 4, "hypothesis_planes: scale must be 1, 2 or 4 (got %d)", scale);
    RCMVS_REQUIRE(H % scale == 0 && W % scale == 0, "hypothesis_planes: H,W must be multiples of scale");
    RCMVS_REQUIRE(prev_depth == nullptr || (hp > 0 && wp > 0), "hypothesis_planes: prev_depth needs hp,wp");
    int h = H / scale, w = W / scale;
    dim3 grid((h * w + 255) / 256, B);
    hipLaunchKernelGGL(planes_kernel, grid, dim3(256), 0, as_stream(stream), prev_depth, depth_values, planes,
                       hp, wp, H, W, scale, D, ratio, ND);
    return launch_status("hypothesis_planes");
}

}
```

rc_mvsnet_amd/ops.py:

```python
import ctypes
import os

import torch

from . import _lib

K1_EVENTS = None
K1_UNIFORM_PLANES = _lib.CONSTANTS["RCMVS_K1_UNIFORM_PLANES"]
K1_FAST_BLEND = _lib.CONSTANTS["RCMVS_K1_FAST_BLEND"]
CONV_EVENTS = None


_FIRST_STREAM = {}


def _multi_stream_allowed():
    return os.environ.get("GPU_MAX_HW_QUEUES") == "1" or os.environ.get("RCMVS_ALLOW_MULTI_STREAM") == "1"


def _stream():
    st = torch.cuda.current_stream()
    key = st.device_index
    first = _FIRST_STREAM.setdefault(key, st.cuda_stream)
    if first != st.cuda_stream and not _multi_stream_allowed():
        raise _lib.RcmvsError(
            f"rc_mvsnet_amd launches on ONE HIP stream per device and process: cuda:{key} started on stream {first:#x}, this call is on "
            f"{st.cuda_stream:#x}.  Two hardware queues of one process give silently wrong results on this platform "
            "(profiles/r6_two_streams.txt); use one stream, or one worker process per stream (rc_mvsnet_amd.sharding), or run the "
            "process with GPU_MAX_HW_QUEUES=1.")
    return ctypes.c_void_p(st.cuda_stream)


def _chk(t, name, dtype=torch.float32):
    if not t.is_cuda:
        raise _lib.RcmvsError(f"{name}: expected a tensor on the GPU (the HIP path has no CPU fallback)")
    if t.dtype != dtype:
        raise _lib.RcmvsError(f"{name}: expected {dtype}, got {t.dtype}")
    if not t.is_contiguous():
        raise _lib.RcmvsError(f"{name}: expected a contiguous tensor")
    return ctypes.c_void_p(t.data_ptr())


def _opt(t, name):
    return ctypes.c_void_p(0) if t is None else _chk(t, name)


def to_channels_last(x):
    N, C = x.shape[:2]
    S = x[0, 0].numel()
    out = torch.empty((N, *x.shape[2:], C), device=x.device, dtype=torch.float32)
    _lib.call("rcmvs_nchw_to_nhwc", _chk(x, "x"), _chk(out, "out"), N, C, S, _stream())
    return out


def to_channels_first(x):
    N, C = x.shape[0], x.shape[-1]
    S = x[0, ..., 0].numel()
    out = torch.empty((N, C, *x.shape[1:-1]), device=x.device, dtype=torch.float32)
    _lib.call("rcmvs_nhwc_to_nchw", _chk(x, "x"), _chk(out, "out"), N, C, S, _stream())
    return out


def compose_homography(proj):
    B, V = proj.shape[:2]
    rot = torch.empty((B, V - 1, 9), device=proj.device, dtype=torch.float32)
    trans = torch.empty((B, V - 1, 3), device=proj.device, dtype=torch.float32)
    _lib.call("rcmvs_compose_homography", _chk(proj, "proj"), _chk(rot, "rot"), _chk(trans, "trans"), B, V, _stream())
    return rot, trans


def compose_homography_stages(projs, zero=None):
    B, V = projs[0].shape[:2]
    n = len(projs)
    rot = torch.empty((n, B, V - 1, 9), device=projs[0].device, dtype=torch.float32)
    trans = torch.empty((n, B, V - 1, 3), device=projs[0].device, dtype=torch.float32)
    ptrs = [_chk(p, "proj") for p in projs] + [ctypes.c_void_p(0)] * (4 - n)
    _lib.call("rcmvs_compose_homography_stages", ptrs[0], ptrs[1], ptrs[2], ptrs[3], n, _chk(rot, "rot"), _chk(trans, "trans"), B, V,
              _opt(zero, "zero"), 0 if zero is None else zero.numel(), _stream())
    return rot, trans


def hypothesis_planes(prev_depth, depth_values, full_hw, scale, ndepth, ratio):
    B, ND = depth_values.shape
    H, W = full_hw
    planes = torch.empty((B, H // scale, W // scale, 2), device=depth_values.device, dtype=torch.float32)
    hp, wp = (prev_depth.shape[-2:] if prev_depth is not None else (0, 0))
    _lib.call("rcmvs_hypothesis_planes", _opt(prev_depth, "prev_depth"), _chk(depth_values, "depth_values"),
              _chk(planes, "planes"), B, hp, wp, H, W, scale, ndepth, float(ratio), ND,
              _stream())
    return planes


ABSMAX_FLOATS = _lib.CONSTANTS["RCMVS_ABSMAX_FLOATS"]


def absmax(x, square=False, out=None):
    if out is None:
        out = torch.zeros(ABSMAX_FLOATS, device=x.device, dtype=torch.float32)
    _lib.call("rcmvs_absmax_fwd", _chk(x, "x"), x.numel(), int(bool(square)), _chk(out, "absmax"), _stream())
    return out


def warp_variance(feats, rot, trans, planes, ndepth, variant=None, uniform_planes=False):
    B, V, h, w, C = feats.shape
    var = torch.empty((B, ndepth, h, w, C), device=feats.device, dtype=torch.float32)
    args = (_chk(feats, "feats"), _chk(rot, "rot"), _chk(trans, "trans"), _chk(planes, "planes"), _chk(var, "var"), B, V, C, ndepth, h, w)
    if variant is not None:
        _lib.call("rcmvs_debug_warp_variance_fwd", *args, int(variant), _stream())
        return var
    hint = K1_FAST_BLEND | (K1_UNIFORM_PLANES if uniform_planes else 0)
    if K1_EVENTS is not None:
        ev = (torch.cuda.Event(enable_timing=True), torch.cuda.Event(enable_timing=True))
        ev[0].record()
        ev[1].record()
        _lib.call("rcmvs_warp_variance_timed_fwd", *args, hint, ctypes.c_void_p(ev[0].cuda_event), ctypes.c_void_p(ev[1].cuda_event), _stream())
        K1_EVENTS.append(ev)
        return var
    _lib.call("rcmvs_warp_variance_hint_fwd", *args, hint, _stream())
    return var


def warp_variance_win(feats, rot, trans, planes, ndepth, variant=5):
    B, V, h, w, C = feats.shape
    var = torch.empty((B, ndepth, h, w, C), device=feats.device, dtype=torch.float32)
    stats = torch.zeros(2, device=feats.device, dtype=torch.int32)
    _lib.call("rcmvs_debug_warp_variance_win_fwd", _chk(feats, "feats"), _chk(rot, "rot"), _chk(trans, "trans"),
              _chk(planes, "planes"), _chk(var, "var"), B, V, C, ndepth, h, w, int(variant),
              _chk(stats, "stats", torch.int32), _stream())
    n = stats.cpu()
    return var, int(n[0]), int(n[1])


def warp_noref(feats, imgs, rot, trans, planes, ndepth, square_first):
    B, V, h, w, C = feats.shape
    out = torch.empty((B, 3 * (V - 1) + C, ndepth, h, w), device=feats.device, dtype=torch.float32)
    _lib.call("rcmvs_warp_noref_fwd", _chk(feats, "feats"), _chk(imgs, "imgs"), _chk(rot, "rot"), _chk(trans, "trans"),
              _chk(planes, "planes"), _chk(out, "out"), B, V, C, ndepth, h, w,
              int(bool(square_first)), _stream())
    return out


def warp_variance_bwd(feats, rot, trans, planes, grad_var, grad_noref=None, variant=0):
    B, V, h, w, C = feats.shape
    D = grad_var.shape[1]
    if tuple(grad_var.shape) != (B, D, h, w, C) or (grad_noref is not None and grad_noref.shape != grad_var.shape):
        raise _lib.RcmvsError(f"warp_variance_bwd: gradient shape {tuple(grad_var.shape)} does not match (B,D,h,w,C)")
    gf = torch.zeros_like(feats)
    args = (_chk(feats, "feats"), _chk(rot, "rot"), _chk(trans, "trans"), _chk(planes, "planes"), _chk(grad_var, "grad_var"),
            _opt(grad_noref, "grad_noref"), _chk(gf, "grad_feats"), B, V, C, D, h, w)
    if variant:
        _lib.call("rcmvs_debug_warp_variance_bwd", *args, int(variant), _stream())
    else:
        _lib.call("rcmvs_warp_variance_bwd", *args, _stream())
    return gf


class WarpVarianceFn(torch.autograd.Function):

    @staticmethod
    def forward(ctx, feats, rot, trans, planes, ndepth, imgs):
        feats = feats.contiguous()
        ctx.save_for_backward(feats, rot, trans, planes)
        ctx.ndepth = ndepth
        ctx.set_materialize_grads(False)
        var = warp_variance(feats, rot, trans, planes, ndepth)
        if imgs is None:
            return var
        noref = warp_noref(feats, imgs, rot, trans, planes, ndepth, square_first=False)
        return var, noref

    @staticmethod
    def backward(ctx, gvar, gnoref=None):
        feats, rot, trans, planes = ctx.saved_tensors
        C = feats.shape[-1]
        if gvar is None and gnoref is None:
            return None, None, None, None, None, None
        if gvar is None:
            gvar = torch.zeros((feats.shape[0], ctx.ndepth, *feats.shape[2:]), device=feats.device)
        gnr = None
        if gnoref is not None:
            gnr = gnoref[:, -C:].permute(0, 2, 3, 4, 1).contiguous()
        gf = warp_variance_bwd(feats, rot, trans, planes, gvar.contiguous(), gnr)
        return gf, None, None, None, None, None


IMG_ALL = 0x7fffffff


class PackedWeight:
    __slots__ = ("blob", "ci", "co", "k", "transposed", "images")

    def __init__(self, blob, ci, co, transposed=0, images=IMG_ALL):
        self.blob, self.ci, self.co, self.transposed, self.images = blob, ci, co, int(transposed), int(images)


_CONV_IMPL = 0


def force_direct_conv(on):
    global _CONV_IMPL
    _CONV_IMPL = int(on)


def _conv_event_start():
    ev = (torch.cuda.Event(enable_timing=True), torch.cuda.Event(enable_timing=True))
    ev[0].record()
    return ev


def _conv_event_stop(ev, *key):
    ev[1].record()
    CONV_EVENTS.append(ev + (key,))


def conv3d_images(ci, co, stride=1, transposed=False, planar=False):
    return int(_lib.load().rcmvs_conv3d_images(co, ci, int(stride), int(bool(transposed)), int(bool(planar))))


def pack_conv3d_weight(w, transposed=False, use=None):
    w = w.detach().contiguous().float()
    Ci, Co = (w.shape[0], w.shape[1]) if transposed else (w.shape[1], w.shape[0])
    n = _lib.load().rcmvs_packed_weight_floats(Co, Ci)
    blob = torch.empty((n,), device=w.device, dtype=torch.float32)
    images = IMG_ALL
    if use is not None and not _CONV_IMPL:
        images = conv3d_images(Ci, Co, stride=use[0], transposed=(int(transposed) == 1), planar=use[1])
    _lib.call("rcmvs_pack_conv3d_weight_sel", _chk(w, "w"), _chk(blob, "packed"), Co, Ci, int(transposed), images, _stream())
    return PackedWeight(blob, Ci, Co, int(transposed), images)


def _check_image(w_packed, ci, co, stride, transposed, planar, scaled, who):
    if w_packed.images == IMG_ALL:
        return
    if _CONV_IMPL or scaled or not (w_packed.images & conv3d_images(ci, co, stride, transposed, planar)):
        raise _lib.RcmvsError(f"{who}: the weight was packed for another call (pack_conv3d_weight(use=...)): the image this call reads was not written")


def conv3d(x, w_packed, scale=None, shift=None, residual=None, stride=1, relu=False, x_absmax=None, y_absmax=None, y_absmax_square=False):
    B, D, H, W, Ci = x.shape
    Co = w_packed.co
    if w_packed.ci != Ci:
        raise _lib.RcmvsError(f"conv3d: input has {Ci} channels, weight expects {w_packed.ci}")
    if w_packed.transposed == 1:
        raise _lib.RcmvsError("conv3d: the weight was packed as a ConvTranspose3d weight (transposed=1); its blob holds no conv images")
    _check_image(w_packed, Ci, Co, stride, False, D == 1, x_absmax is not None, "conv3d")
    y = torch.empty((B, (D - 1) // stride + 1, (H - 1) // stride + 1, (W - 1) // stride + 1, Co), device=x.device,
                    dtype=torch.float32)
    if residual is not None and residual.shape != y.shape:
        raise _lib.RcmvsError(f"conv3d: residual {tuple(residual.shape)} != output {tuple(y.shape)}")
    ev = _conv_event_start() if CONV_EVENTS is not None else None
    if x_absmax is not None or y_absmax is not None:
        name, xb, yb = "rcmvs_conv3d_scaled_fwd", (_opt(x_absmax, "x_absmax"),), (_opt(y_absmax, "y_absmax"),)
        impl = (_CONV_IMPL | ((1 << 24) if y_absmax_square else 0),)
    elif _CONV_IMPL:
        name, xb, yb, impl = "rcmvs_debug_conv3d_fwd", (), (), (_CONV_IMPL,)
    else:
        name, xb, yb, impl = "rcmvs_conv3d_fwd", (), (), ()
    _lib.call(name, _chk(x, "x"), *xb, _chk(w_packed.blob, "w"), _opt(scale, "scale"), _opt(shift, "shift"), _opt(residual, "residual"),
              _chk(y, "y"), *yb, B, D, H, W, Ci, Co, stride, int(relu), *impl, _stream())
    if ev is not None:
        _conv_event_stop(ev, "s1" if stride == 1 else "s2", B, D, H, W, Ci, Co)
    return y


def deconv3d(x, w_packed, scale=None, shift=None, residual=None, relu=False, x_absmax=None, y_absmax=None):
    B, D, H, W, Ci = x.shape
    Co = w_packed.co
    if w_packed.ci != Ci:
        raise _lib.RcmvsError(f"deconv3d: input has {Ci} channels, weight expects {w_packed.ci}")
    if w_packed.transposed != 1:
        raise _lib.RcmvsError("deconv3d: the weight was not packed with transposed=True; its blob holds no transposed-conv image")
    _check_image(w_packed, Ci, Co, 2, True, False, x_absmax is not None, "deconv3d")
    y = torch.empty((B, 2 * D, 2 * H, 2 * W, Co), device=x.device, dtype=torch.float32)
    if residual is not None and residual.shape != y.shape:
        raise _lib.RcmvsError(f"deconv3d: residual {tuple(residual.shape)} != output {tuple(y.shape)} "
                              "(volume sizes must be divisible by 8, as in the reference)")
    ev = _conv_event_start() if CONV_EVENTS is not None else None
    if x_absmax is not None or y_absmax is not None:
        name, xb, yb, impl = "rcmvs_deconv3d_scaled_fwd", (_opt(x_absmax, "x_absmax"),), (_opt(y_absmax, "y_absmax"),), (_CONV_IMPL,)
    elif _CONV_IMPL:
        name, xb, yb, impl = "rcmvs_debug_deconv3d_fwd", (), (), (_CONV_IMPL,)
    else:
        name, xb, yb, impl = "rcmvs_deconv3d_fwd", (), (), ()
    _lib.call(name, _chk(x, "x"), *xb, _chk(w_packed.blob, "w"), _opt(scale, "scale"), _opt(shift, "shift"), _opt(residual, "residual"),
              _chk(y, "y"), *yb, B, D, H, W, Ci, Co, int(relu), *impl, _stream())
    if ev is not None:
        _conv_event_stop(ev, "t2", B, D, H, W, Ci, Co)
    return y


def conv2d_s2d(x, w_packed, scale=None, shift=None, relu=False):
    N, H, W, C = x.shape
    Co = w_packed.co
    if w_packed.ci != 4 * C:
        raise _lib.RcmvsError(f"conv2d_s2d: input has {C} channels, the packed weight expects {w_packed.ci} = 4 x C")
    y = torch.empty((N, H // 2, W // 2, Co), device=x.device, dtype=torch.float32)
    _lib.call("rcmvs_conv2d_s2d_fwd", _chk(x, "x"), _chk(w_packed.blob, "w"), _opt(scale, "scale"), _opt(shift, "shift"),
              _chk(y, "y"), N, H, W, C, Co, int(relu), _stream())
    return y


def pack_conv2d_pair(wa, wb):
    if tuple(wa.shape) != (16, 16, 3, 3) or tuple(wb.shape) != (16, 16, 3, 3):
        raise _lib.RcmvsError("pack_conv2d_pair: built for two 16 -> 16 3x3 layers")
    lib = _lib.load()
    img = torch.empty(int(lib.rcmvs_conv2d_pair_weight_floats()), device=wa.device, dtype=torch.float32)
    _lib.call("rcmvs_pack_conv2d_pair", _chk(wa.detach().float().contiguous(), "wa"), _chk(wb.detach().float().contiguous(), "wb"), _chk(img, "image"), _stream())
    return img


def conv2d_pair(x, image, scale_a, shift_a, scale_b, shift_b):
    N, H, W, C = x.shape
    y = torch.empty_like(x)
    _lib.call("rcmvs_conv2d_pair_fwd", _chk(x, "x"), _chk(image, "image"), _chk(scale_a, "scale_a"), _chk(shift_a, "shift_a"),
              _chk(scale_b, "scale_b"), _chk(shift_b, "shift_b"), _chk(y, "y"), N, H, W, C, _stream())
    return y


def resize_rgb_cl(x, hw):
    N, C, H, W = x.shape
    if C != 3:
        raise _lib.RcmvsError("resize_rgb_cl: expects RGB images (N,3,H,W)")
    h, w = int(hw[0]), int(hw[1])
    y = torch.empty((N, h, w, 3), device=x.device, dtype=torch.float32)
    _lib.call("rcmvs_resize_rgb_cl", _chk(x, "x"), _chk(y, "y"), N, H, W, h, w, _stream())
    return y


def rgb_to_nhwc4(x):
    N, _, H, W = x.shape
    y = torch.empty((N, H, W, 4), device=x.device, dtype=torch.float32)
    _lib.call("rcmvs_rgb_to_nhwc4", _chk(x, "x"), _chk(y, "y"), N, H, W, _stream())
    return y


def pack_conv2d_weight(w, pad_in_to=None):
    w = w.detach().contiguous().float()
    Co, Ci, K, _ = w.shape
    Cip = Ci if pad_in_to is None else pad_in_to
    blob = torch.empty((K * K * Cip * Co,), device=w.device, dtype=torch.float32)
    _lib.call("rcmvs_pack_conv2d_weight", _chk(w, "w"), _chk(blob, "packed"), Co, Ci, Cip, K, _stream())
    pw = PackedWeight(blob, Cip, Co)
    pw.k = K
    return pw


def conv2d(x, w_packed, scale=None, shift=None, up_add=None, stride=1, relu=False):
    N, H, W, Ci = x.shape
    K, Co = w_packed.k, w_packed.co
    if w_packed.ci != Ci:
        raise _lib.RcmvsError(f"conv2d: input has {Ci} channels, weight expects {w_packed.ci}")
    Ho, Wo = (H + 2 * (K // 2) - K) // stride + 1, (W + 2 * (K // 2) - K) // stride + 1
    y = torch.empty((N, Ho, Wo, Co), device=x.device, dtype=torch.float32)
    if up_add is not None and tuple(up_add.shape) != (N, Ho // 2, Wo // 2, Co):
        raise _lib.RcmvsError(f"conv2d: up_add {tuple(up_add.shape)} does not match half of the output {tuple(y.shape)}")
    _lib.call("rcmvs_conv2d_fwd", _chk(x, "x"), _chk(w_packed.blob, "w"), _opt(scale, "scale"), _opt(shift, "shift"),
              _opt(up_add, "up_add"), _chk(y, "y"), N, H, W, Ci, Co, K, stride, int(relu), _stream())
    return y


def conv1x1(x, w_packed, scale=None, shift=None, up_add=None, relu=False, ysq_absmax=None, mfma=False):
    N, H, W, Ci = x.shape
    Co = w_packed.co
    if w_packed.ci != Ci or w_packed.k != 1:
        raise _lib.RcmvsError(f"conv1x1: input has {Ci} channels, weight is {w_packed.ci} -> {Co} with k={w_packed.k}")
    if up_add is not None and tuple(up_add.shape) != (N, H // 2, W // 2, Co):
        raise _lib.RcmvsError(f"conv1x1: up_add {tuple(up_add.shape)} does not match half of the output")
    y = torch.empty((N, H, W, Co), device=x.device, dtype=torch.float32)
    _lib.call("rcmvs_conv1x1_mfma_fwd" if mfma else "rcmvs_conv1x1_fwd", _chk(x, "x"), _chk(w_packed.blob, "w"), _opt(scale, "scale"), _opt(shift, "shift"),
              _opt(up_add, "up_add"), _chk(y, "y"), _opt(ysq_absmax, "ysq_absmax"), N, H, W, Ci, Co, int(relu), _stream())
    return y


def conv2d_rgb(x, w_packed, scale=None, shift=None, relu=False):
    N, C, H, W = x.shape
    if C != 3 or w_packed.ci != 4 or w_packed.co != 8 or w_packed.k != 3:
        raise _lib.RcmvsError(f"conv2d_rgb: expected a (N,3,H,W) input and a 3 -> 8 3x3 weight packed to 4 input channels (got {tuple(x.shape)}, {w_packed.ci} -> {w_packed.co}, k={w_packed.k})")
    y = torch.empty((N, H, W, 8), device=x.device, dtype=torch.float32)
    _lib.call("rcmvs_conv2d_fwd", _chk(x, "x"), _chk(w_packed.blob, "w"), _opt(scale, "scale"), _opt(shift, "shift"), None,
              _chk(y, "y"), N, H, W, 3, 8, 3, 1, int(relu), _stream())
    return y


def pack_conv2d_tile(w):
    Co = w.shape[0]
    if Co not in (16, 32) or tuple(w.shape) != (Co, 32, 3, 3):
        raise _lib.RcmvsError("pack_conv2d_tile: built for 32 -> 16 and 32 -> 32 3x3 layers")
    lib = _lib.load()
    img = torch.empty(int(lib.rcmvs_conv2d_tile_weight_floats(Co)), device=w.device, dtype=torch.float32)
    _lib.call("rcmvs_pack_conv2d_tile", _chk(w.detach().float().contiguous(), "w"), _chk(img, "image"), Co, _stream())
    return img


def conv2d_tile(x, image, scale=None, shift=None, relu=False, s2d=False, ysq_absmax=None):
    N, Hx, Wx, C = x.shape
    lib = _lib.load()
    Co = {int(lib.rcmvs_conv2d_tile_weight_floats(c)): c for c in (16, 32)}.get(image.numel())
    if Co is None or C != (8 if s2d else 32) or (s2d and (Hx % 2 or Wx % 2 or Co != 16)):
        raise _lib.RcmvsError(f"conv2d_tile: unexpected input {tuple(x.shape)} (s2d={s2d}) or image of {image.numel()} floats")
    H, W = (Hx // 2, Wx // 2) if s2d else (Hx, Wx)
    y = torch.empty((N, H, W, Co), device=x.device, dtype=torch.float32)
    _lib.call("rcmvs_conv2d_tile_fwd", _chk(x, "x"), _chk(image, "image"), _opt(scale, "scale"), _opt(shift, "shift"), _chk(y, "y"), N, H, W, Co, int(s2d), int(relu),
              _opt(ysq_absmax, "ysq_absmax"), _stream())
    return y


def pack_conv2d_stem(wb):
    if tuple(wb.shape) != (8, 8, 3, 3):
        raise _lib.RcmvsError("pack_conv2d_stem: built for an 8 -> 8 3x3 second layer")
    lib = _lib.load()
    img = torch.empty(int(lib.rcmvs_conv2d_stem_weight_floats()), device=wb.device, dtype=torch.float32)
    _lib.call("rcmvs_pack_conv2d_stem", _chk(wb.detach().float().contiguous(), "wb"), _chk(img, "image"), _stream())
    return img


def conv2d_stem(x, w_a_packed, scale_a, shift_a, image_b, scale_b, shift_b):
    N, C, H, W = x.shape
    if C != 3 or w_a_packed.ci != 4 or w_a_packed.co != 8 or w_a_packed.k != 3:
        raise _lib.RcmvsError(f"conv2d_stem: expected a (N,3,H,W) input and a 3 -> 8 3x3 weight packed to 4 input channels (got {tuple(x.shape)}, {w_a_packed.ci} -> {w_a_packed.co}, k={w_a_packed.k})")
    y = torch.empty((N, H, W, 8), device=x.device, dtype=torch.float32)
    _lib.call("rcmvs_conv2d_stem_fwd", _chk(x, "x"), _chk(w_a_packed.blob, "w_a"), _chk(scale_a, "scale_a"), _chk(shift_a, "shift_a"), _chk(image_b, "image_b"),
              _chk(scale_b, "scale_b"), _chk(shift_b, "shift_b"), _chk(y, "y"), N, H, W, _stream())
    return y


def fpn_out_fused(lat, up, w_inner_packed, b_inner, w_out_packed):
    N, H, W, CL = lat.shape
    CM, CO = w_inner_packed.co, w_out_packed.co
    if w_inner_packed.ci != CL or w_inner_packed.k != 1 or w_out_packed.ci != CM or w_out_packed.k != 3:
        raise _lib.RcmvsError("fpn_out_fused: expected a 1x1 lateral conv followed by a 3x3 output conv on matching channels")
    if tuple(up.shape) != (N, H // 2, W // 2, CM):
        raise _lib.RcmvsError(f"fpn_out_fused: up {tuple(up.shape)} does not match half of {tuple(lat.shape)} with {CM} channels")
    y = torch.empty((N, H, W, CO), device=lat.device, dtype=torch.float32)
    _lib.call("rcmvs_fpn_out_fused", _chk(lat, "lat"), _chk(up, "up"), _chk(w_inner_packed.blob, "w_inner"), _chk(b_inner, "b_inner"),
              _chk(w_out_packed.blob, "w_out"), _chk(y, "y"), N, H, W, CL, CM, CO, _stream())
    return y


FPN_FOLDED_FLOATS = _lib.CONSTANTS["RCMVS_FPN_FOLDED_FLOATS"]


def pack_fpn_folded(w_inner, b_inner, w_out):
    wi = w_inner.detach().double().reshape(32, 8)
    wo = w_out.detach().double()
    b = b_inner.detach().double()
    wb = torch.einsum("mi,omyx->yxio", wi, wo)
    bt = torch.einsum("m,omyx->yxo", b, wo)
    inside = {0: (1, 2), 1: (0, 1, 2), 2: (0, 1)}
    bs = torch.stack([torch.stack([sum(bt[ky, kx] for ky in inside[cy] for kx in inside[cx]) for cx in range(3)]) for cy in range(3)])
    rows = lambda p: ((0,), (1, 2)) if p == 0 else ((0, 1), (2,))
    wa = torch.zeros(2, 2, 2, 2, 32, 8, dtype=torch.float64, device=wo.device)
    for py in range(2):
        for px in range(2):
            for ry in range(2):
                for rx in range(2):
                    for ky in rows(py)[ry]:
                        for kx in rows(px)[rx]:
                            wa[py, px, ry, rx] += wo[:, :, ky, kx].t()
    tab = torch.cat((wb.reshape(-1), bs.reshape(-1), wa.reshape(-1))).float().contiguous()
    assert tab.numel() == FPN_FOLDED_FLOATS
    return tab


def pack_fpn_folded_mfma(tables):
    if tables.numel() != FPN_FOLDED_FLOATS:
        raise _lib.RcmvsError("pack_fpn_folded_mfma: expects the tables of pack_fpn_folded")
    img = torch.empty((_lib.load().rcmvs_fpn_folded_mfma_floats(),), device=tables.device, dtype=torch.float32)
    _lib.call("rcmvs_fpn_folded_mfma_pack", _chk(tables, "tables"), _chk(img, "image"), _stream())
    return img


def fpn_out_folded(lat, up, tables, ysq_absmax=None):
    N, H, W, CL = lat.shape
    mfma = tables.numel() == _lib.load().rcmvs_fpn_folded_mfma_floats()
    if CL != 8 or tuple(up.shape) != (N, H // 2, W // 2, 32) or not (mfma or tables.numel() == FPN_FOLDED_FLOATS):
        raise _lib.RcmvsError(f"fpn_out_folded: lat {tuple(lat.shape)} / up {tuple(up.shape)} / {tables.numel()} table floats do not fit 8 -> 32 -> 8")
    y = torch.empty((N, H, W, 8), device=lat.device, dtype=torch.float32)
    _lib.call("rcmvs_fpn_out_folded_mfma" if mfma else "rcmvs_fpn_out_folded", _chk(lat, "lat"), _chk(up, "up"), _chk(tables, "tables"), _chk(y, "y"),
              _opt(ysq_absmax, "ysq_absmax"), N, H, W, _stream())
    return y


DEPTH_HEAD_IMPL = 0


def depth_head(x8, w_prob_packed, planes, want_prob=False, x_absmax=None):
    B, D, h, w, C = x8.shape
    if C != 8:
        raise _lib.RcmvsError("depth_head: the prob conv takes 8 channels")
    if x_absmax is not None and w_prob_packed.images != IMG_ALL:
        raise _lib.RcmvsError("depth_head: the fp16-pair form reads an image that a selectively packed weight does not hold")
    depth = torch.empty((B, h, w), device=x8.device, dtype=torch.float32)
    conf = torch.empty((B, h, w), device=x8.device, dtype=torch.float32)
    one_launch = D == 8 and not (DEPTH_HEAD_IMPL & 1)
    prob = None if one_launch and not want_prob else torch.empty((B, D, h, w), device=x8.device, dtype=torch.float32)
    _lib.call("rcmvs_depth_head_scaled_fwd", _chk(x8, "x8"), _opt(x_absmax, "x_absmax"), _chk(w_prob_packed.blob, "w_prob"), _chk(planes, "planes"),
              _chk(depth, "depth"), _chk(conf, "conf"), _opt(prob, "prob"), B, D, h, w,
              DEPTH_HEAD_IMPL | (0 if want_prob else 8), _stream())
    return (depth, conf, prob) if want_prob else (depth, conf)


def conv11_prob(t, t_absmax, w11_packed, scale, shift, res, res_absmax, coef, w_prob_packed, zchunk=0, planes=None):
    B, Dt, Ht, Wt, C = t.shape
    if C != 16 or tuple(res.shape) != (B, 2 * Dt, 2 * Ht, 2 * Wt, 8):
        raise _lib.RcmvsError(f"conv11_prob: t {tuple(t.shape)} / res {tuple(res.shape)} are not (B,Dt,Ht,Wt,16) / (B,2Dt,2Ht,2Wt,8)")
    if w11_packed.images != IMG_ALL or w_prob_packed.images != IMG_ALL:
        raise _lib.RcmvsError("conv11_prob: needs the full weight blobs (a selectively packed weight does not hold the fp16-pair images)")
    fused = planes is not None and Dt == 4
    logits = depth = conf = None
    if fused:
        depth = torch.empty((B, 2 * Ht, 2 * Wt), device=t.device, dtype=torch.float32)
        conf = torch.empty((B, 2 * Ht, 2 * Wt), device=t.device, dtype=torch.float32)
    else:
        logits = torch.empty((B, 2 * Dt, 2 * Ht, 2 * Wt), device=t.device, dtype=torch.float32)
    _lib.call("rcmvs_conv11_prob_fwd", _chk(t, "t"), _chk(t_absmax, "t_absmax"), _chk(w11_packed.blob, "w11"), _chk(scale, "scale"),
              _chk(shift, "shift"), _chk(res, "res"), _chk(res_absmax, "res_absmax"), _chk(coef, "coef"),
              _chk(w_prob_packed.blob, "w_prob"), _opt(logits, "logits"), _opt(planes if fused else None, "planes"),
              _opt(depth, "depth"), _opt(conf, "conf"), B, Dt, Ht, Wt, int(zchunk), _stream())
    if fused:
        return depth, conf
    if planes is not None:
        return softmax_head(logits, planes)
    return logits


def softmax_head(logits, planes, keep_prob=False):
    B, D, h, w = logits.shape
    depth = torch.empty((B, h, w), device=logits.device, dtype=torch.float32)
    conf = torch.empty((B, h, w), device=logits.device, dtype=torch.float32)
    _lib.call("rcmvs_softmax_head_fwd", _chk(logits, "logits"), _chk(planes, "planes"), _chk(depth, "depth"), _chk(conf, "conf"),
              B, D, h, w, int(bool(keep_prob)), _stream())
    return depth, conf


def resize_planes(x, out_planes, pad_channels_to=None):
    B, C, D, h, w = x.shape
    Cp = C if pad_channels_to is None else pad_channels_to
    y = torch.empty((B, out_planes, h, w, Cp), device=x.device, dtype=torch.float32)
    _lib.call("rcmvs_resize_planes_fwd", _chk(x, "x"), _chk(y, "y"), B, C, Cp, D, out_planes, h, w, _stream())
    return y


def gu_sample(pseudo_depth, img0, pix, eps, u, cam):
    H, W = pseudo_depth.shape
    N, S = eps.shape
    dev = eps.device
    f = lambda *shape: torch.empty(shape, device=dev, dtype=torch.float32)
    z, pts, ndc, dirs, rdepth, target = f(N, S), f(N, S, 3), f(N, S, 3), f(N, 3), f(N), f(N, 3)
    _lib.call("rcmvs_gu_sample_fwd", _chk(pseudo_depth, "pseudo_depth"), _chk(img0, "img0"), _chk(pix, "pix", torch.int32),
              _chk(eps, "eps"), _chk(u, "u"), _chk(cam, "cam"), _chk(z, "z"), _chk(pts, "pts"),
              _chk(ndc, "ndc"), _chk(dirs, "dirs"), _chk(rdepth, "rays_depth"), _chk(target, "target"),
              N, S, H, W, _stream())
    return z, pts, ndc, dirs, rdepth, target


def point_feats(volume_cl, imgs, poses, pts, ndc, ldf=32):
    Dv, hv, wv, C = volume_cl.shape
    if C != 8:
        raise _lib.RcmvsError("point_feats: the neural volume has 8 channels")
    nimg, _, H, W = imgs.shape
    M = pts.shape[0] * pts.shape[1]
    feat = torch.empty((M, ldf), device=pts.device, dtype=torch.float32)
    _lib.call("rcmvs_point_feats_fwd", _chk(volume_cl, "volume"), _chk(imgs, "imgs"), _chk(poses, "poses"), _chk(pts, "pts"),
              _chk(ndc, "ndc"), _chk(feat, "feat"), M, Dv, hv, wv, nimg, H, W, ldf, _stream())
    return feat


NERF_ORDER = ("pts_bias", "pts_linears.0", "pts_linears.1", "pts_linears.2", "pts_linears.3", "pts_linears.4", "pts_linears.5",
              "alpha_linear", "feature_linear", "views_linears.0", "rgb_linear")


def pack_nerf_weights(named):
    lib = _lib.load()
    tensors = []
    for n in NERF_ORDER:
        w, b = named[n]
        tensors += [w.detach().contiguous().float(), b.detach().contiguous().float()]
    arr = (ctypes.c_void_p * 22)(*[_chk(t, "nerf weight").value for t in tensors])
    blob = torch.empty((lib.rcmvs_nerf_weight_floats(),), device=tensors[0].device, dtype=torch.float32)
    _lib.call("rcmvs_pack_nerf_weights", arr, _chk(blob, "blob"), _stream())
    return blob


def nerf_mlp(ndc, feat, dirs, w2c_ref, blob):
    lib = _lib.load()
    N, S = ndc.shape[:2]
    M = N * S
    ws = torch.empty((lib.rcmvs_nerf_workspace_floats(M),), device=ndc.device, dtype=torch.float32)
    raw = torch.empty((N, S, 4), device=ndc.device, dtype=torch.float32)
    _lib.call("rcmvs_nerf_mlp_fwd", _chk(ndc, "ndc"), _chk(feat, "feat"), feat.shape[1], _chk(dirs, "dirs"), _chk(w2c_ref, "w2c_ref"),
              _chk(blob, "weights"), _chk(ws, "workspace"), _chk(raw, "raw"), N, S, _stream())
    return raw


def nerf_mlp_embedded(x, blob):
    lib = _lib.load()
    M, ldx = x.shape
    if ldx != 86:
        raise _lib.RcmvsError(f"nerf_mlp_embedded: rows of 63 + 20 + 3 = 86 columns expected (got {ldx})")
    ws = torch.empty((lib.rcmvs_nerf_workspace_floats(M),), device=x.device, dtype=torch.float32)
    feat = torch.empty((M, 32), device=x.device, dtype=torch.float32)
    raw = torch.empty((M, 4), device=x.device, dtype=torch.float32)
    _lib.call("rcmvs_nerf_mlp_embedded_fwd", _chk(x, "x"), ldx, _chk(blob, "weights"), _chk(ws, "workspace"), _chk(feat, "feat"), _chk(raw, "raw"), M, _stream())
    return raw


def composite(raw, z):
    N, S = z.shape
    dev = z.device
    rgb = torch.empty((N, 3), device=dev, dtype=torch.float32)
    depth = torch.empty((N,), device=dev, dtype=torch.float32)
    weights = torch.empty((N, S), device=dev, dtype=torch.float32)
    alpha = torch.empty((N, S), device=dev, dtype=torch.float32)
    _lib.call("rcmvs_composite_fwd", _chk(raw, "raw"), _chk(z, "z"), _chk(rgb, "rgb"), _chk(depth, "depth"),
              _chk(weights, "weights"), _chk(alpha, "alpha"), N, S, _stream())
    return rgb, depth, weights, alpha
```

Baseline: 965.4 ref-scenes/s.

## Fuse next-stage hypothesis plane computation into depth heads and homography compose

The softmax/depth-head kernels now compute the next stage's hypothesis-plane table in the same launch. Each tile keeps its depth in shared memory with a one-pixel halo and bilinearly upsamples it to derive the refined planes. Stage 1's plane table comes out of the homography-compose launch. Together these remove the separate hypothesis_planes launches and the re-read of the depth map.

The 1x1 conv MFMA path now prefetches the up-add operand together with the input and supports odd map sizes. A new opt-in flag (off by default) routes the inner1 lateral conv through the MFMA 1x1 kernel. The fused head recomputes halo softmax columns, which adds some redundant work in exchange for fewer launches.

```diff
diff --git a/rc_mvsnet_amd/_lib.py b/rc_mvsnet_amd/_lib.py
--- a/rc_mvsnet_amd/_lib.py
+++ b/rc_mvsnet_amd/_lib.py
@@ -8,6 +8,7 @@
 LIB_PATH = os.path.join(_HERE, "librcmvs_hip.so")
 CSRC = os.path.join(_HERE, "csrc")
 HEADER = os.path.join(os.path.dirname(_HERE), "include", "rcmvs.h")
+EXT_HEADER = os.path.join(CSRC, "rcmvs_planes.h")
 
 _lib = None
 
@@ -88,6 +89,8 @@
 
 
 SIGNATURES, _RESTYPES, CONSTANTS = parse_header(_read_header())
+with open(EXT_HEADER) as _f:
+    EXT_SIGNATURES = parse_header(_f.read())[0]
 REQUIRED_VERSION = CONSTANTS["RCMVS_VERSION"]
 
 
@@ -132,7 +135,7 @@
         raise RcmvsError(f"{path} is missing: run `python -c 'import __graft_entry__ as g; g.build()'` "
                          "(hipcc --offload-arch=gfx950). There is no CPU / eager fallback.")
     lib = ctypes.CDLL(path)
-    for name, argtypes in SIGNATURES.items():
+    for name, argtypes in list(SIGNATURES.items()) + list(EXT_SIGNATURES.items()):
         fn = getattr(lib, name)
         fn.argtypes = argtypes
         fn.restype = _RESTYPES.get(name, ctypes.c_int)
diff --git a/rc_mvsnet_amd/casmvsnet.py b/rc_mvsnet_amd/casmvsnet.py
--- a/rc_mvsnet_amd/casmvsnet.py
+++ b/rc_mvsnet_amd/casmvsnet.py
@@ -7,6 +7,8 @@
 CONV_TILE = os.environ.get("RCMVS_CONV_TILE", "1") != "0"
 CONV_STEM = os.environ.get("RCMVS_CONV_STEM", "1") != "0"
 CONV_PAIR = os.environ.get("RCMVS_CONV_PAIR", "1") != "0"
+LATERAL_MFMA = os.environ.get("RCMVS_LATERAL_MFMA", "0") != "0"
+SIDE_PLANES = os.environ.get("RCMVS_SIDE_PLANES", "1") != "0"
 DEEP_PAIR = os.environ.get("RCMVS_DEEP_PAIR", "1") != "0"
 
 import torch
@@ -299,7 +301,10 @@
                 out["stage3"] = plain(lambda t=intra: one(t, "out3"))
             return out if lazy else {k: f()[0] for k, f in out.items()}
         if self.num_stage >= 2:
-            intra = ops.conv2d(c1, p["inner1"][0], None, p["inner1"][1], up_add=c2)
+            if LATERAL_MFMA and p["inner1"][0].ci == 16 and p["inner1"][0].co == 32:
+                intra = ops.conv1x1(c1, p["inner1"][0], None, p["inner1"][1], up_add=c2, mfma=True)
+            else:
+                intra = ops.conv2d(c1, p["inner1"][0], None, p["inner1"][1], up_add=c2)
             if isinstance(p["out2"], tuple):
                 def out2(bound=None, t=intra):
                     keep = bound is not None and not ops._CONV_IMPL
@@ -506,7 +511,7 @@
         c2 = shift.abs().max() * (1.0 + 2.0 ** -10)
         return torch.stack((c1, c2)).float().contiguous()
 
-    def features_cl(self, x, x_absmax=None, plan=None, logits=False, planes=None):
+    def features_cl(self, x, x_absmax=None, plan=None, logits=False, planes=None, next_stage=None):
         B, D, h, w, _ = x.shape
         if D % 8 or h % 8 or w % 8:
             raise RcmvsError(f"CostRegNet: volume {D}x{h}x{w} must be divisible by 8 in every axis "
@@ -539,7 +544,7 @@
             t = ops.deconv3d(t, *p["conv7"], residual=conv4, relu=True, y_absmax=b[5])
         t = ops.deconv3d(t, *p["conv9"], residual=conv2, relu=True, x_absmax=b[5], y_absmax=b[4])
         if logits:
-            return ops.conv11_prob(t, b[4], p["conv11"][0], p["conv11"][1], p["conv11"][2], conv0, b[0], p["conv11_coef"], p["prob"], planes=planes)
+            return ops.conv11_prob(t, b[4], p["conv11"][0], p["conv11"][1], p["conv11"][2], conv0, b[0], p["conv11_coef"], p["prob"], planes=planes, next_stage=next_stage)
         return ops.deconv3d(t, *p["conv11"], residual=conv0, relu=True, x_absmax=b[4], y_absmax=b[9])
 
     def features_cl_train(self, x):
@@ -689,10 +694,17 @@
                 bounds = self._pair_bounds = torch.zeros(self.num_stage, CostRegNet.BOUND_ROWS, ops.ABSMAX_FLOATS, device=imgs.device, dtype=torch.float32)
             else:
                 need_fill = True
+        side_planes = SIDE_PLANES and homographies is None and self.num_stage <= 4
+        next_planes = None
         if homographies is None:
             if self.num_stage <= 4:
-                rots, transs = ops.compose_homography_stages([proj_matrices["stage{}".format(k + 1)].contiguous().float() for k in range(self.num_stage)],
-                                                             zero=bounds if need_fill else None)
+                projs = [proj_matrices["stage{}".format(k + 1)].contiguous().float() for k in range(self.num_stage)]
+                if side_planes:
+                    scale0 = int(self.stage_infos["stage1"]["scale"])
+                    rots, transs, next_planes = ops.compose_homography_stages(projs, zero=bounds if need_fill else None,
+                                                                              planes=(depth_values, (H // scale0, W // scale0), self.ndepths[0]))
+                else:
+                    rots, transs = ops.compose_homography_stages(projs, zero=bounds if need_fill else None)
                 need_fill = False
             else:
                 rt = [ops.compose_homography(proj_matrices["stage{}".format(k + 1)].contiguous().float()) for k in range(self.num_stage)]
@@ -715,7 +727,15 @@
                 rot, trans = homographies[key]
             else:
                 rot, trans = rots[s], transs[s]
-            planes = ops.hypothesis_planes(depth, depth_values, (H, W), scale, D, self.depth_interals_ratio[s])
+            if next_planes is not None:
+                planes, next_planes = next_planes, None
+            else:
+                planes = ops.hypothesis_planes(depth, depth_values, (H, W), scale, D, self.depth_interals_ratio[s])
+            nxt = None
+            if side_planes and s + 1 < self.num_stage:
+                scale_n = int(self.stage_infos["stage{}".format(s + 2)]["scale"])
+                if H == 2 * h * scale_n and W == 2 * w * scale_n:
+                    nxt = (depth_values, (H, W), scale_n, self.ndepths[s + 1], self.depth_interals_ratio[s + 1])
             var = ops.warp_variance(f_cl, rot, trans, planes, D, uniform_planes=depth is None)
             cr = self._cr(s)
             vmax = None
@@ -725,10 +745,15 @@
                     ops.absmax(f_cl, square=True, out=vmax[0])
             plan = cr.hip_plan()
             if vmax is not None and HEAD_PAIR and (CONV11_PROB == 2 or (CONV11_PROB == 1 and D == 8)):
-                depth, conf = cr.features_cl(var, vmax, plan, logits=True, planes=planes)
+                res = cr.features_cl(var, vmax, plan, logits=True, planes=planes, next_stage=nxt if D != 8 else None)
             else:
                 x8 = cr.features_cl(var, vmax, plan)
-                depth, conf = ops.depth_head(x8, plan["prob"], planes, x_absmax=vmax[CostRegNet.BOUND_ROWS - 1] if vmax is not None and HEAD_PAIR else None)
+                head_pair = vmax is not None and HEAD_PAIR
+                res = ops.depth_head(x8, plan["prob"], planes, x_absmax=vmax[CostRegNet.BOUND_ROWS - 1] if head_pair else None,
+                                     next_stage=nxt if head_pair and D != 8 else None)
+            depth, conf = res[:2]
+            if len(res) == 3:
+                next_planes = res[2]
             out = {"depth": depth, "photometric_confidence": conf}
             if self.TRAIN_VARIANT:
                 small_cl = ops.resize_rgb_cl(imgs.reshape(B * V, 3, H, W).contiguous(), (h, w)).view(B, V, h, w, 3)
diff --git a/rc_mvsnet_amd/csrc/conv2d.hip b/rc_mvsnet_amd/csrc/conv2d.hip
--- a/rc_mvsnet_amd/csrc/conv2d.hip
+++ b/rc_mvsnet_amd/csrc/conv2d.hip
@@ -175,7 +175,7 @@
             const long long hw = (long long)H * W;
             const long long n = p / hw;
             const int r = (int)(p - n * hw), oy = r / W, ox = r - oy * W;
-            const float* upp = up + ((n * (H / 2) + oy / 2) * (W / 2) + ox / 2) * CO;
+            const float* upp = up + ((n * ((H + 1) / 2) + oy / 2) * ((W + 1) / 2) + ox / 2) * CO;
 #pragma unroll
             for (int co = 0; co < CO; co += 4) {
                 const f4v u4 = *reinterpret_cast<const f4v*>(upp + co);
@@ -300,17 +300,24 @@
         else return __builtin_amdgcn_mfma_f32_16x16x16bf16_1k(__builtin_bit_cast(s16x4, a), __builtin_bit_cast(s16x4, b), c, 0, 0, 0);
     };
     const long long ntiles = (npix + 15) / 16, stride = (long long)gridDim.x * 4;
-    x3_f32x4 xq[KL / 4];
+    const long long hw = (long long)H * W;
+    x3_f32x4 xq[KL / 4], uq[2] = {(x3_f32x4){0.f, 0.f, 0.f, 0.f}, (x3_f32x4){0.f, 0.f, 0.f, 0.f}};
     auto fetch = [&](long long tile) {
         const long long p = tile * 16 + n;
         const bool in = tile < ntiles && p < npix;
 #pragma unroll
         for (int c = 0; c < KL / 4; ++c) xq[c] = in ? *reinterpret_cast<const x3_f32x4*>(x + p * CI + kq * KL + c * 4) : (x3_f32x4){0.f, 0.f, 0.f, 0.f};
+        if (up && in) {
+            const long long b = p / hw;
+            const int r = (int)(p - b * hw), oy = r / W, ox = r - oy * W;
+            const float* upp = up + ((b * ((H + 1) / 2) + oy / 2) * ((W + 1) / 2) + ox / 2) * CO + kq * 4;
+            uq[0] = *reinterpret_cast<const x3_f32x4*>(upp);
+            uq[1] = *reinterpret_cast<const x3_f32x4*>(upp + 16);
+        }
     };
     float vmax = 0.0f;
     long long tile = (long long)blockIdx.x * 4 + wave;
     fetch(tile);
-    const long long hw = (long long)H * W;
     for (; tile < ntiles; tile += stride) {
         frag_t bq[3];
         {
@@ -322,15 +329,10 @@
                 bq[0] = (frag_t){h0.x, h0.y, h1.x, h1.y}; bq[1] = (frag_t){m0.x, m0.y, m1.x, m1.y}; bq[2] = (frag_t){l0.x, l0.y, l1.x, l1.y};
             } else { bq[0] = (frag_t){h0.x, h0.y}; bq[1] = (frag_t){m0.x, m0.y}; bq[2] = (frag_t){l0.x, l0.y}; }
         }
+        const x3_f32x4 ua[2] = {uq[0], uq[1]};
         fetch(tile + stride);
         const long long p = tile * 16 + n;
         const bool live = p < npix;
-        long long upo = 0;
-        if (up && live) {
-            const long long b = p / hw;
-            const int r = (int)(p - b * hw), oy = r / W, ox = r - oy * W;
-            upo = ((b * (H / 2) + oy / 2) * (W / 2) + ox / 2) * CO;
-        }
 #pragma unroll
         for (int mt = 0; mt < 2; ++mt) {
             x3_f32x4 acc[3] = {(x3_f32x4){0.f, 0.f, 0.f, 0.f}, (x3_f32x4){0.f, 0.f, 0.f, 0.f}, (x3_f32x4){0.f, 0.f, 0.f, 0.f}};
@@ -345,7 +347,7 @@
             if (scale) v = v * *reinterpret_cast<const x3_f32x4*>(scale + co);
             if (shift) v = v + *reinterpret_cast<const x3_f32x4*>(shift + co);
             if (live) {
-                if (up) v = *reinterpret_cast<const x3_f32x4*>(up + upo + co) + v;
+                if (up) v = ua[mt] + v;
                 if (relu) v = __builtin_elementwise_max(v, (x3_f32x4){0.f, 0.f, 0.f, 0.f});
                 *reinterpret_cast<x3_f32x4*>(y + p * CO + co) = v;
                 vmax = x3_absmax4(vmax, v);
@@ -397,7 +399,6 @@
                       float* y, float* ysq_absmax, int N, int H, int W, int Ci, int Co, int relu, void* stream) {
     RCMVS_REQUIRE(x && w_packed && y, "conv1x1_fwd: null pointer");
     RCMVS_REQUIRE(N > 0 && H > 0 && W > 0, "conv1x1_fwd: bad sizes");
-    RCMVS_REQUIRE(!up_add || (H % 2 == 0 && W % 2 == 0), "conv1x1_fwd: the up-add merge needs even H and W (got %d x %d)", H, W);
     hipStream_t st = as_stream(stream);
     if (Ci == 16 && Co == 32) return conv1x1_launch_t<16, 32>(x, w_packed, scale, shift, up_add, y, ysq_absmax, N, H, W, relu, st);
     if (Ci == 32 && Co == 32) return conv1x1_launch_t<32, 32>(x, w_packed, scale, shift, up_add, y, ysq_absmax, N, H, W, relu, st);
@@ -409,7 +410,6 @@
                            float* y, float* ysq_absmax, int N, int H, int W, int Ci, int Co, int relu, void* stream) {
     RCMVS_REQUIRE(x && w_packed && y, "conv1x1_mfma_fwd: null pointer");
     RCMVS_REQUIRE(N > 0 && H > 0 && W > 0, "conv1x1_mfma_fwd: bad sizes");
-    RCMVS_REQUIRE(!up_add || (H % 2 == 0 && W % 2 == 0), "conv1x1_mfma_fwd: the up-add merge needs even H and W (got %d x %d)", H, W);
     hipStream_t st = as_stream(stream);
     if (Ci == 16 && Co == 32) return conv1x1_mfma_launch_t<16>(x, w_packed, scale, shift, up_add, y, ysq_absmax, N, H, W, relu, st);
     if (Ci == 32 && Co == 32) return conv1x1_mfma_launch_t<32>(x, w_packed, scale, shift, up_add, y, ysq_absmax, N, H, W, relu, st);
diff --git a/rc_mvsnet_amd/csrc/depth_head.hip b/rc_mvsnet_amd/csrc/depth_head.hip
--- a/rc_mvsnet_amd/csrc/depth_head.hip
+++ b/rc_mvsnet_amd/csrc/depth_head.hip
@@ -1,4 +1,5 @@
 #include "common.h"
+#include "plane_math.h"
 
 namespace rcmvs {
 
@@ -12,15 +13,9 @@
 int prob_head_fused_launch(const float* x, const float* wp, const float* planes, float* depth, float* conf, float* prob,
                            int B, int D, int H, int W, hipStream_t st);
 
-template <int LP, bool KEEP = true>
-__global__ __launch_bounds__(256) void softmax_regress_kernel(float* __restrict__ prob, const float* __restrict__ planes,
-                                                               float* __restrict__ depth, float* __restrict__ conf, int D, long long hw) {
+template <int LP, bool KEEP>
+__device__ static inline void softmax_column(float* __restrict__ col, const float2 pl, int D, long long hw, int j, bool live, float& depth, float& conf) {
     constexpr int MAXK = 16;
-    const int b = blockIdx.y;
-    const int j = threadIdx.x % LP;
-    const long long p = ((long long)blockIdx.x * blockDim.x + threadIdx.x) / LP;
-    const bool live = p < hw;
-    float* col = prob + (long long)b * D * hw + (live ? p : 0);
     float v[MAXK];
     float mx = -INFINITY;
 #pragma unroll
@@ -39,7 +34,6 @@
     }
 #pragma unroll
     for (int m = 1; m < LP; m <<= 1) sum += __shfl_xor(sum, m);
-    const float2 pl = reinterpret_cast<const float2*>(planes)[(long long)b * hw + (live ? p : 0)];
     float dsum = 0.0f, isum = 0.0f;
 #pragma unroll
     for (int i = 0; i < MAXK; ++i) {
@@ -63,18 +57,108 @@
     }
 #pragma unroll
     for (int m = 1; m < LP; m <<= 1) c += __shfl_xor(c, m);
+    depth = dsum;
+    conf = c;
+}
+
+template <int LP, bool KEEP = true>
+__global__ __launch_bounds__(256) void softmax_regress_kernel(float* __restrict__ prob, const float* __restrict__ planes,
+                                                               float* __restrict__ depth, float* __restrict__ conf, int D, long long hw) {
+    const int b = blockIdx.y;
+    const int j = threadIdx.x % LP;
+    const long long p = ((long long)blockIdx.x * blockDim.x + threadIdx.x) / LP;
+    const bool live = p < hw;
+    float* col = prob + (long long)b * D * hw + (live ? p : 0);
+    const float2 pl = reinterpret_cast<const float2*>(planes)[(long long)b * hw + (live ? p : 0)];
+    float dsum, c;
+    softmax_column<LP, KEEP>(col, pl, D, hw, j, live, dsum, c);
     if (live && j == 0) {
         depth[(long long)b * hw + p] = dsum;
         conf[(long long)b * hw + p] = c;
     }
 }
 
+template <int LP, int RH, int RW>
+__global__ __launch_bounds__(256) void softmax_regress_planes_kernel(const float* __restrict__ logits, const float* __restrict__ planes,
+                                                                      float* __restrict__ depth, float* __restrict__ conf, int D, int h, int w, int tiles_w,
+                                                                      const float* __restrict__ dv, float* __restrict__ next, int H, int W, int scale, int Dn, float ratio, int ND) {
+    constexpr int TH = RH - 2, TW = RW - 2, SLOTS = 256 / LP;
+    static_assert((RH * RW) % SLOTS == 0, "whole passes over the region");
+    __shared__ float sd[RH * RW];
+    const int b = blockIdx.y;
+    const int ty0 = (blockIdx.x / tiles_w) * TH, tx0 = (blockIdx.x % tiles_w) * TW;
+    const int j = threadIdx.x % LP;
+    const long long hw = (long long)h * w;
+    for (int slot = threadIdx.x / LP; slot < RH * RW; slot += SLOTS) {
+        const int ry = slot / RW, rx = slot % RW;
+        const int gy = ty0 - 1 + ry, gx = tx0 - 1 + rx;
+        const bool live = gy >= 0 && gy < h && gx >= 0 && gx < w;
+        const long long p = live ? (long long)gy * w + gx : 0;
+        float* col = const_cast<float*>(logits) + (long long)b * D * hw + p;
+        const float2 pl = reinterpret_cast<const float2*>(planes)[(long long)b * hw + p];
+        float dsum, c;
+        softmax_column<LP, false>(col, pl, D, hw, j, live, dsum, c);
+        if (live && j == 0) {
+            sd[slot] = dsum;
+            if (ry >= 1 && ry <= TH && rx >= 1 && rx <= TW) {
+                depth[(long long)b * hw + p] = dsum;
+                conf[(long long)b * hw + p] = c;
+            }
+        }
+    }
+    __syncthreads();
+    const int hn = H / scale, wn = W / scale;
+    const float sh = (float)h / (float)H, sw = (float)w / (float)W;
+    constexpr int CH = 2 * TH + 1, CW = 2 * TW + 1;
+    float2* out = reinterpret_cast<float2*>(next) + (long long)b * hn * wn;
+    for (int c = threadIdx.x; c < CH * CW; c += 256) {
+        const int y = 2 * ty0 + c / CW, x = 2 * tx0 + c % CW;
+        if (y >= hn || x >= wn) continue;
+        const UpTaps t = up_taps(h, w, sh, sw, plane_first_tap(y, scale), plane_first_tap(x, scale));
+        if (t.y0 < ty0 || t.y0 >= ty0 + TH || t.x0 < tx0 || t.x0 >= tx0 + TW) continue;
+        out[(long long)y * wn + x] = refined_plane([&](int yy, int xx) { return sd[(yy - ty0 + 1) * RW + (xx - tx0 + 1)]; },
+                                                   dv, h, w, H, W, scale, Dn, ratio, ND, y, x);
+    }
+}
+
 }
 
 using namespace rcmvs;
 
+struct NextPlanes { const float* dv; float* planes; int H, W, scale, D; float ratio; int ND; };
+
+static int softmax_launch(float* prob, const float* planes, float* depth, float* conf, int B, int D, int h, int w, bool keep, const NextPlanes* np, hipStream_t st) {
+    const long long hw = (long long)h * w;
+    if (np) {
+#define RCMVS_SOFTMAX_PLANES(LP, RH, RW) do { const int tw = (int)cdiv(w, RW - 2), th = (int)cdiv(h, RH - 2); \
+        hipLaunchKernelGGL((softmax_regress_planes_kernel<LP, RH, RW>), dim3((unsigned)(tw * th), B), dim3(256), 0, st, prob, planes, depth, conf, D, h, w, tw, \
+                           np->dv, np->planes, np->H, np->W, np->scale, np->D, np->ratio, np->ND); } while (0)
+        if (D <= 16) RCMVS_SOFTMAX_PLANES(1, 16, 16);
+        else if (D <= 32) RCMVS_SOFTMAX_PLANES(2, 16, 16);
+        else RCMVS_SOFTMAX_PLANES(4, 8, 16);
+#undef RCMVS_SOFTMAX_PLANES
+        return 0;
+    }
+#define RCMVS_SOFTMAX(LP) do { if (keep) hipLaunchKernelGGL((softmax_regress_kernel<LP, true>), dim3((unsigned)cdiv(hw * LP, 256), B), dim3(256), 0, st, prob, planes, depth, conf, D, hw); \
+                               else hipLaunchKernelGGL((softmax_regress_kernel<LP, false>), dim3((unsigned)cdiv(hw * LP, 256), B), dim3(256), 0, st, prob, planes, depth, conf, D, hw); } while (0)
+    if (D <= 16) RCMVS_SOFTMAX(1);
+    else if (D <= 32) RCMVS_SOFTMAX(2);
+    else RCMVS_SOFTMAX(4);
+#undef RCMVS_SOFTMAX
+    return 0;
+}
+
+static int next_planes_check(const NextPlanes& np, int h, int w, const char* who) {
+    RCMVS_REQUIRE(np.dv && np.planes, "%s: null pointer (depth_values, next_planes)", who);
+    RCMVS_REQUIRE(np.H > 0 && np.W > 0 && np.D >= 2 && np.ND >= 2, "%s: bad sizes of the next stage", who);
+    RCMVS_REQUIRE(np.scale == 1 || np.scale == 2 || np.scale == 4, "%s: the next stage's scale must be 1, 2 or 4 (got %d)", who, np.scale);
+    RCMVS_REQUIRE(np.H == 2 * h * np.scale && np.W == 2 * w * np.scale, "%s: the next stage's table (%d x %d / %d) must be twice the %d x %d map in each axis",
+                  who, np.H, np.W, np.scale, h, w);
+    return 0;
+}
+
 static int depth_head_fwd(const float* x, const float* xmax, const float* w_prob, const float* planes, float* depth, float* conf, float* prob,
-                          int B, int D, int h, int w, int impl, void* stream) {
+                          int B, int D, int h, int w, int impl, void* stream, const NextPlanes* np = nullptr) {
     RCMVS_REQUIRE(x && w_prob && planes && depth && conf, "depth_head_fwd: null pointer");
     RCMVS_REQUIRE(B > 0 && D > 0 && h > 0 && w > 0, "depth_head_fwd: bad sizes");
     RCMVS_REQUIRE(D <= 64, "depth_head_fwd: at most 64 depth hypotheses per stage (got %d)", D);
@@ -82,21 +166,18 @@
     const int zc_force = (impl >> 8) & 0xff;
     const bool pair = xmax && !(impl & 4) && prob_pair_supported(D, h, w);
     int rc;
-    if (pair && D == 8 && !(impl & 1))
+    if (np) {
+        RCMVS_REQUIRE(impl & 8, "depth_head_planes_fwd: the probabilities cannot be kept (impl bit 3 must be set: the logits are read by neighbouring blocks)");
+        if ((rc = next_planes_check(*np, h, w, "depth_head_planes_fwd"))) return rc;
+    }
+    if (!np && pair && D == 8 && !(impl & 1))
         return prob_pair_launch(x, w_prob + prob_pair_blob_offset(), xmax, prob, planes, depth, conf, B, D, h, w, true, 0, st);
-    if (!pair && !(impl & 1) && prob_head_fused_supported(D, h, w)) return prob_head_fused_launch(x, w_prob, planes, depth, conf, prob, B, D, h, w, st);
+    if (!np && !pair && !(impl & 1) && prob_head_fused_supported(D, h, w)) return prob_head_fused_launch(x, w_prob, planes, depth, conf, prob, B, D, h, w, st);
     RCMVS_REQUIRE(prob, "depth_head_fwd: prob is required for D = %d (it doubles as the logit scratch; only the D = 8 form runs without)", D);
     if (pair) rc = prob_pair_launch(x, w_prob + prob_pair_blob_offset(), xmax, prob, nullptr, nullptr, nullptr, B, D, h, w, false, zc_force, st);
     else rc = conv3d_lds_launch(x, w_prob, nullptr, nullptr, nullptr, prob, B, D, h, w, 8, 1, 0, st, ((impl & 2) ? 16 : 0) | (zc_force << 8));
     if (rc) return rc;
-    const long long hw = (long long)h * w;
-    const bool keep = !(impl & 8);
-#define RCMVS_SOFTMAX(LP) do { if (keep) hipLaunchKernelGGL((softmax_regress_kernel<LP, true>), dim3((unsigned)cdiv(hw * LP, 256), B), dim3(256), 0, st, prob, planes, depth, conf, D, hw); \
-                               else hipLaunchKernelGGL((softmax_regress_kernel<LP, false>), dim3((unsigned)cdiv(hw * LP, 256), B), dim3(256), 0, st, prob, planes, depth, conf, D, hw); } while (0)
-    if (D <= 16) RCMVS_SOFTMAX(1);
-    else if (D <= 32) RCMVS_SOFTMAX(2);
-    else RCMVS_SOFTMAX(4);
-#undef RCMVS_SOFTMAX
+    softmax_launch(prob, planes, depth, conf, B, D, h, w, !(impl & 8), np, st);
     return launch_status("depth_head_fwd");
 }
 
@@ -104,15 +185,20 @@
     RCMVS_REQUIRE(prob && planes && depth && conf, "softmax_head_fwd: null pointer");
     RCMVS_REQUIRE(B > 0 && D > 0 && h > 0 && w > 0, "softmax_head_fwd: bad sizes");
     RCMVS_REQUIRE(D <= 64, "softmax_head_fwd: at most 64 depth hypotheses per stage (got %d)", D);
-    hipStream_t st = as_stream(stream);
-    const long long hw = (long long)h * w;
-#define RCMVS_SOFTMAX(LP) do { if (keep) hipLaunchKernelGGL((softmax_regress_kernel<LP, true>), dim3((unsigned)cdiv(hw * LP, 256), B), dim3(256), 0, st, prob, planes, depth, conf, D, hw); \
-                               else hipLaunchKernelGGL((softmax_regress_kernel<LP, false>), dim3((unsigned)cdiv(hw * LP, 256), B), dim3(256), 0, st, prob, planes, depth, conf, D, hw); } while (0)
-    if (D <= 16) RCMVS_SOFTMAX(1);
-    else if (D <= 32) RCMVS_SOFTMAX(2);
-    else RCMVS_SOFTMAX(4);
-#undef RCMVS_SOFTMAX
+    softmax_launch(prob, planes, depth, conf, B, D, h, w, keep != 0, nullptr, as_stream(stream));
     return launch_status("softmax_head_fwd");
+}
+
+extern "C" int rcmvs_softmax_head_planes_fwd(const float* logits, const float* planes, float* depth, float* conf, int B, int D, int h, int w,
+                                             const float* depth_values, float* next_planes, int H, int W, int next_scale, int next_D, float next_ratio, int ND,
+                                             void* stream) {
+    RCMVS_REQUIRE(logits && planes && depth && conf, "softmax_head_planes_fwd: null pointer");
+    RCMVS_REQUIRE(B > 0 && D > 0 && h > 0 && w > 0, "softmax_head_planes_fwd: bad sizes");
+    RCMVS_REQUIRE(D <= 64, "softmax_head_planes_fwd: at most 64 depth hypotheses per stage (got %d)", D);
+    const NextPlanes np{depth_values, next_planes, H, W, next_scale, next_D, next_ratio, ND};
+    if (int rc = next_planes_check(np, h, w, "softmax_head_planes_fwd")) return rc;
+    softmax_launch(const_cast<float*>(logits), planes, depth, conf, B, D, h, w, false, &np, as_stream(stream));
+    return launch_status("softmax_head_planes_fwd");
 }
 
 extern "C" int rcmvs_depth_head_fwd(const float* x, const float* w_prob, const float* planes, float* depth, float* conf, float* prob,
@@ -123,3 +209,9 @@
                                            float* prob, int B, int D, int h, int w, int impl, void* stream) {
     return depth_head_fwd(x, x_absmax, w_prob, planes, depth, conf, prob, B, D, h, w, impl, stream);
 }
+extern "C" int rcmvs_depth_head_planes_fwd(const float* x, const float* x_absmax, const float* w_prob, const float* planes, float* depth, float* conf,
+                                           float* prob, int B, int D, int h, int w, int impl, const float* depth_values, float* next_planes,
+                                           int H, int W, int next_scale, int next_D, float next_ratio, int ND, void* stream) {
+    const NextPlanes np{depth_values, next_planes, H, W, next_scale, next_D, next_ratio, ND};
+    return depth_head_fwd(x, x_absmax, w_prob, planes, depth, conf, prob, B, D, h, w, impl, stream, &np);
+}
diff --git a/rc_mvsnet_amd/csrc/geometry.hip b/rc_mvsnet_amd/csrc/geometry.hip
--- a/rc_mvsnet_amd/csrc/geometry.hip
+++ b/rc_mvsnet_amd/csrc/geometry.hip
@@ -1,4 +1,5 @@
 #include "common.h"
+#include "plane_math.h"
 
 namespace rcmvs {
 
@@ -82,13 +83,20 @@
 
 struct ProjPtrs { const float* p[4]; };
 __global__ void compose_homography_kernel(ProjPtrs pp, float* __restrict__ rot,
-                                          float* __restrict__ trans, int B, int V, float* __restrict__ zero, int zero_n) {
-    for (int i = (blockIdx.y * gridDim.x + blockIdx.x) * blockDim.x + threadIdx.x; i < zero_n; i += gridDim.x * gridDim.y * blockDim.x) zero[i] = 0.0f;
-    int t = blockIdx.x * blockDim.x + threadIdx.x;
+                                          float* __restrict__ trans, int B, int V, int hb, int nstage, float* __restrict__ zero, int zero_n,
+                                          const float* __restrict__ dv, float* __restrict__ planes, int planes_n, int D, int ND) {
+    for (int i = blockIdx.x * blockDim.x + threadIdx.x; i < zero_n; i += gridDim.x * blockDim.x) zero[i] = 0.0f;
+    const int stage = blockIdx.x / hb;
+    if (stage >= nstage) {
+        const long long e = (long long)(blockIdx.x - nstage * hb) * blockDim.x + threadIdx.x;
+        if (e < (long long)B * planes_n) reinterpret_cast<float2*>(planes)[e] = uniform_plane(dv, (int)(e / planes_n), D, ND);
+        return;
+    }
+    int t = (blockIdx.x - stage * hb) * blockDim.x + threadIdx.x;
     if (t >= B * (V - 1)) return;
-    const float* proj = pp.p[blockIdx.y];
-    rot += (long long)blockIdx.y * B * (V - 1) * 9;
-    trans += (long long)blockIdx.y * B * (V - 1) * 3;
+    const float* proj = pp.p[stage];
+    rot += (long long)stage * B * (V - 1) * 9;
+    trans += (long long)stage * B * (V - 1) * 3;
     int b = t / (V - 1), v = 1 + t % (V - 1);
     double R[4][4], S[4][4], inv[4][4];
     fold_intrinsics(proj + ((long long)b * V + 0) * 32, R);
@@ -132,64 +140,21 @@
 #endif
 }
 
-__device__ static inline float bilinear_up(const float* __restrict__ p, int hp, int wp, float sh, float sw, int Y, int X) {
-#pragma clang fp contract(off)
-    float sy = sh * ((float)Y + 0.5f) - 0.5f;
-    float sx = sw * ((float)X + 0.5f) - 0.5f;
-    sy = sy < 0.f ? 0.f : sy;
-    sx = sx < 0.f ? 0.f : sx;
-    int y0 = (int)sy, x0 = (int)sx;
-    y0 = y0 > hp - 1 ? hp - 1 : y0;
-    x0 = x0 > wp - 1 ? wp - 1 : x0;
-    int y1 = y0 + 1 > hp - 1 ? hp - 1 : y0 + 1;
-    int x1 = x0 + 1 > wp - 1 ? wp - 1 : x0 + 1;
-    float ly1 = sy - (float)y0, lx1 = sx - (float)x0;
-    float ly0 = 1.0f - ly1, lx0 = 1.0f - lx1;
-    float top = lx0 * ld_agent(p + y0 * wp + x0) + lx1 * ld_agent(p + y0 * wp + x1);
-    float bot = lx0 * ld_agent(p + y1 * wp + x0) + lx1 * ld_agent(p + y1 * wp + x1);
-    return ly0 * top + ly1 * bot;
-}
-
 __global__ __launch_bounds__(256) void planes_kernel(const float* __restrict__ prev, const float* __restrict__ dv,
                                                       float* __restrict__ planes, int hp, int wp, int H, int W,
                                                       int scale, int D, float ratio, int ND) {
-#pragma clang fp contract(off)
     const int h = H / scale, w = W / scale;
     const int b = blockIdx.y;
     int t = blockIdx.x * blockDim.x + threadIdx.x;
     if (t >= h * w) return;
     int y = t / w, x = t % w;
-    float d0, delta;
+    float2 o;
     if (prev == nullptr) {
-        float lo = dv[(long long)b * ND], hi = dv[(long long)b * ND + ND - 1];
-        d0 = lo;
-        delta = (hi - lo) / (float)(D - 1);
+        o = uniform_plane(dv, b, D, ND);
     } else {
-        double itv = ((double)dv[ND - 1] - (double)dv[0]) / (double)ND;
-        float half = (float)((double)D / 2.0 * ((double)ratio * itv));
         const float* p = prev + (long long)b * hp * wp;
-        float sh = (float)hp / (float)H, sw = (float)wp / (float)W;
-        float fd = (float)(D - 1);
-        if (scale == 1) {
-            float c = bilinear_up(p, hp, wp, sh, sw, y, x);
-            float cmin = c - half, cmax = c + half;
-            d0 = cmin;
-            delta = (cmax - cmin) / fd;
-        } else {
-            int Y0 = y * scale + scale / 2 - 1, X0 = x * scale + scale / 2 - 1;
-            float mn[2][2], it[2][2];
-            for (int j = 0; j < 2; ++j)
-                for (int i = 0; i < 2; ++i) {
-                    float c = bilinear_up(p, hp, wp, sh, sw, Y0 + j, X0 + i);
-                    float cmin = c - half, cmax = c + half;
-                    mn[j][i] = cmin;
-                    it[j][i] = (cmax - cmin) / fd;
-                }
-            d0 = 0.5f * (0.5f * mn[0][0] + 0.5f * mn[0][1]) + 0.5f * (0.5f * mn[1][0] + 0.5f * mn[1][1]);
-            delta = 0.5f * (0.5f * it[0][0] + 0.5f * it[0][1]) + 0.5f * (0.5f * it[1][0] + 0.5f * it[1][1]);
-        }
-    }
-    float2 o = make_float2(d0, delta);
+        o = refined_plane([p, wp](int yy, int xx) { return ld_agent(p + yy * wp + xx); }, dv, hp, wp, H, W, scale, D, ratio, ND, y, x);
+    }
     reinterpret_cast<float2*>(planes)[(long long)b * h * w + t] = o;
 }
 
@@ -214,20 +179,34 @@
     RCMVS_REQUIRE(B > 0 && V >= 2 && V - 1 <= RCMVS_MAX_SRC_VIEWS, "compose_homography: B=%d V=%d", B, V);
     const int n = B * (V - 1);
     ProjPtrs pp{{proj, nullptr, nullptr, nullptr}};
-    hipLaunchKernelGGL(compose_homography_kernel, dim3((n + 63) / 64), dim3(64), 0, as_stream(stream), pp, rot, trans, B, V, (float*)nullptr, 0);
+    hipLaunchKernelGGL(compose_homography_kernel, dim3((n + 63) / 64), dim3(64), 0, as_stream(stream), pp, rot, trans, B, V, (n + 63) / 64, 1, (float*)nullptr, 0,
+                       (const float*)nullptr, (float*)nullptr, 0, 0, 0);
     return launch_status("compose_homography");
 }
 
-int rcmvs_compose_homography_stages(const float* proj0, const float* proj1, const float* proj2, const float* proj3, int nstage,
-                                    float* rot, float* trans, int B, int V, float* zero, long long zero_n, void* stream) {
+int rcmvs_compose_homography_stages_planes(const float* proj0, const float* proj1, const float* proj2, const float* proj3, int nstage,
+                                           float* rot, float* trans, int B, int V, float* zero, long long zero_n,
+                                           const float* depth_values, float* planes, long long planes_n, int D, int ND, void* stream) {
     RCMVS_REQUIRE(zero_n >= 0 && zero_n < (1LL << 24) && (zero || zero_n == 0), "compose_homography_stages: bad side buffer (%lld floats)", zero_n);
     RCMVS_REQUIRE(rot && trans && nstage >= 1 && nstage <= 4, "compose_homography_stages: bad arguments (1..4 stages)");
     RCMVS_REQUIRE(B > 0 && V >= 2 && V - 1 <= RCMVS_MAX_SRC_VIEWS, "compose_homography_stages: B=%d V=%d", B, V);
+    RCMVS_REQUIRE(planes_n >= 0 && (planes_n == 0 || (planes && depth_values)), "compose_homography_stages: a plane table needs depth_values and planes");
+    RCMVS_REQUIRE(planes_n == 0 || (D >= 2 && ND >= 2), "compose_homography_stages: the plane table needs D >= 2 and ND >= 2 (got %d, %d)", D, ND);
+    RCMVS_REQUIRE(planes_n * B < (1LL << 28), "compose_homography_stages: plane table of %lld x %d pixels is too large for a side job", planes_n, B);
     ProjPtrs pp{{proj0, proj1, proj2, proj3}};
     for (int s = 0; s < nstage; ++s) RCMVS_REQUIRE(pp.p[s], "compose_homography_stages: stage %d has no projection tensor", s);
     const int n = B * (V - 1);
-    hipLaunchKernelGGL(compose_homography_kernel, dim3((n + 63) / 64, nstage), dim3(zero_n ? 256 : 64), 0, as_stream(stream), pp, rot, trans, B, V, zero, (int)zero_n);
+    const int block = (zero_n || planes_n) ? 256 : 64;
+    const int hb = (n + block - 1) / block;
+    const int table_blocks = (int)cdiv(planes_n * B, block);
+    hipLaunchKernelGGL(compose_homography_kernel, dim3(hb * nstage + table_blocks), dim3(block), 0, as_stream(stream), pp, rot, trans, B, V, hb, nstage, zero, (int)zero_n,
+                       depth_values, planes, (int)planes_n, D, ND);
     return launch_status("compose_homography_stages");
+}
+
+int rcmvs_compose_homography_stages(const float* proj0, const float* proj1, const float* proj2, const float* proj3, int nstage,
+                                    float* rot, float* trans, int B, int V, float* zero, long long zero_n, void* stream) {
+    return rcmvs_compose_homography_stages_planes(proj0, proj1, proj2, proj3, nstage, rot, trans, B, V, zero, zero_n, nullptr, nullptr, 0, 0, 0, stream);
 }
 
 int rcmvs_hypothesis_planes(const float* prev_depth, const float* depth_values, float* planes,
diff --git a/rc_mvsnet_amd/csrc/plane_math.h b/rc_mvsnet_amd/csrc/plane_math.h
--- /dev/null
+++ b/rc_mvsnet_amd/csrc/plane_math.h
@@ -0,0 +1,76 @@
+#pragma once
+#include "common.h"
+#include "rcmvs_planes.h"
+
+namespace rcmvs {
+
+__device__ static inline float2 uniform_plane(const float* __restrict__ dv, int b, int D, int ND) {
+#pragma clang fp contract(off)
+    float lo = dv[(long long)b * ND], hi = dv[(long long)b * ND + ND - 1];
+    return make_float2(lo, (hi - lo) / (float)(D - 1));
+}
+
+struct UpTaps {
+    int y0, x0, y1, x1;
+    float ly0, ly1, lx0, lx1;
+};
+
+__device__ static inline UpTaps up_taps(int hp, int wp, float sh, float sw, int Y, int X) {
+#pragma clang fp contract(off)
+    float sy = sh * ((float)Y + 0.5f) - 0.5f;
+    float sx = sw * ((float)X + 0.5f) - 0.5f;
+    sy = sy < 0.f ? 0.f : sy;
+    sx = sx < 0.f ? 0.f : sx;
+    UpTaps t;
+    t.y0 = (int)sy; t.x0 = (int)sx;
+    t.y0 = t.y0 > hp - 1 ? hp - 1 : t.y0;
+    t.x0 = t.x0 > wp - 1 ? wp - 1 : t.x0;
+    t.y1 = t.y0 + 1 > hp - 1 ? hp - 1 : t.y0 + 1;
+    t.x1 = t.x0 + 1 > wp - 1 ? wp - 1 : t.x0 + 1;
+    t.ly1 = sy - (float)t.y0; t.lx1 = sx - (float)t.x0;
+    t.ly0 = 1.0f - t.ly1; t.lx0 = 1.0f - t.lx1;
+    return t;
+}
+
+template <class Fetch>
+__device__ static inline float bilinear_up(Fetch ld, int hp, int wp, float sh, float sw, int Y, int X) {
+#pragma clang fp contract(off)
+    const UpTaps t = up_taps(hp, wp, sh, sw, Y, X);
+    float top = t.lx0 * ld(t.y0, t.x0) + t.lx1 * ld(t.y0, t.x1);
+    float bot = t.lx0 * ld(t.y1, t.x0) + t.lx1 * ld(t.y1, t.x1);
+    return t.ly0 * top + t.ly1 * bot;
+}
+
+__device__ static inline int plane_first_tap(int y, int scale) { return scale == 1 ? y : y * scale + scale / 2 - 1; }
+
+template <class Fetch>
+__device__ static inline float2 refined_plane(Fetch ld, const float* __restrict__ dv, int hp, int wp, int H, int W, int scale,
+                                              int D, float ratio, int ND, int y, int x) {
+#pragma clang fp contract(off)
+    double itv = ((double)dv[ND - 1] - (double)dv[0]) / (double)ND;
+    float half = (float)((double)D / 2.0 * ((double)ratio * itv));
+    float sh = (float)hp / (float)H, sw = (float)wp / (float)W;
+    float fd = (float)(D - 1);
+    float d0, delta;
+    if (scale == 1) {
+        float c = bilinear_up(ld, hp, wp, sh, sw, y, x);
+        float cmin = c - half, cmax = c + half;
+        d0 = cmin;
+        delta = (cmax - cmin) / fd;
+    } else {
+        int Y0 = plane_first_tap(y, scale), X0 = plane_first_tap(x, scale);
+        float mn[2][2], it[2][2];
+        for (int j = 0; j < 2; ++j)
+            for (int i = 0; i < 2; ++i) {
+                float c = bilinear_up(ld, hp, wp, sh, sw, Y0 + j, X0 + i);
+                float cmin = c - half, cmax = c + half;
+                mn[j][i] = cmin;
+                it[j][i] = (cmax - cmin) / fd;
+            }
+        d0 = 0.5f * (0.5f * mn[0][0] + 0.5f * mn[0][1]) + 0.5f * (0.5f * mn[1][0] + 0.5f * mn[1][1]);
+        delta = 0.5f * (0.5f * it[0][0] + 0.5f * it[0][1]) + 0.5f * (0.5f * it[1][0] + 0.5f * it[1][1]);
+    }
+    return make_float2(d0, delta);
+}
+
+}
diff --git a/rc_mvsnet_amd/csrc/rcmvs_planes.h b/rc_mvsnet_amd/csrc/rcmvs_planes.h
--- /dev/null
+++ b/rc_mvsnet_amd/csrc/rcmvs_planes.h
@@ -0,0 +1,24 @@
+#ifndef RCMVS_PLANES_H
+#define RCMVS_PLANES_H
+
+#ifdef __cplusplus
+extern "C" {
+#endif
+
+int rcmvs_compose_homography_stages_planes(const float* proj0, const float* proj1, const float* proj2, const float* proj3, int nstage,
+                                           float* rot, float* trans, int B, int V, float* zero, long long zero_n,
+                                           const float* depth_values, float* planes, long long planes_n, int D, int ND, void* stream);
+
+int rcmvs_softmax_head_planes_fwd(const float* logits, const float* planes, float* depth, float* conf, int B, int D, int h, int w,
+                                  const float* depth_values, float* next_planes, int H, int W, int next_scale, int next_D, float next_ratio, int ND,
+                                  void* stream);
+int rcmvs_depth_head_planes_fwd(const float* x, const float* x_absmax, const float* w_prob, const float* planes,
+                                float* depth, float* conf, float* prob, int B, int D, int h, int w, int impl,
+                                const float* depth_values, float* next_planes, int H, int W, int next_scale, int next_D, float next_ratio, int ND,
+                                void* stream);
+
+#ifdef __cplusplus
+}
+#endif
+
+#endif
diff --git a/rc_mvsnet_amd/ops.py b/rc_mvsnet_amd/ops.py
--- a/rc_mvsnet_amd/ops.py
+++ b/rc_mvsnet_amd/ops.py
@@ -69,15 +69,24 @@
     return rot, trans
 
 
-def compose_homography_stages(projs, zero=None):
+def compose_homography_stages(projs, zero=None, planes=None):
     B, V = projs[0].shape[:2]
     n = len(projs)
     rot = torch.empty((n, B, V - 1, 9), device=projs[0].device, dtype=torch.float32)
     trans = torch.empty((n, B, V - 1, 3), device=projs[0].device, dtype=torch.float32)
     ptrs = [_chk(p, "proj") for p in projs] + [ctypes.c_void_p(0)] * (4 - n)
-    _lib.call("rcmvs_compose_homography_stages", ptrs[0], ptrs[1], ptrs[2], ptrs[3], n, _chk(rot, "rot"), _chk(trans, "trans"), B, V,
-              _opt(zero, "zero"), 0 if zero is None else zero.numel(), _stream())
-    return rot, trans
+    if planes is None:
+        _lib.call("rcmvs_compose_homography_stages", ptrs[0], ptrs[1], ptrs[2], ptrs[3], n, _chk(rot, "rot"), _chk(trans, "trans"), B, V,
+                  _opt(zero, "zero"), 0 if zero is None else zero.numel(), _stream())
+        return rot, trans
+    depth_values, (h, w), ndepth = planes
+    if depth_values.shape[0] != B:
+        raise _lib.RcmvsError(f"compose_homography_stages: depth_values {tuple(depth_values.shape)} is not (B = {B}, ND)")
+    table = torch.empty((B, h, w, 2), device=projs[0].device, dtype=torch.float32)
+    _lib.call("rcmvs_compose_homography_stages_planes", ptrs[0], ptrs[1], ptrs[2], ptrs[3], n, _chk(rot, "rot"), _chk(trans, "trans"), B, V,
+              _opt(zero, "zero"), ctypes.c_longlong(0 if zero is None else zero.numel()), _chk(depth_values, "depth_values"), _chk(table, "planes"), ctypes.c_longlong(h * w),
+              int(ndepth), depth_values.shape[1], _stream())
+    return rot, trans, table
 
 
 def hypothesis_planes(prev_depth, depth_values, full_hw, scale, ndepth, ratio):
@@ -364,8 +373,8 @@
     Co = w_packed.co
     if w_packed.ci != Ci or w_packed.k != 1:
         raise _lib.RcmvsError(f"conv1x1: input has {Ci} channels, weight is {w_packed.ci} -> {Co} with k={w_packed.k}")
-    if up_add is not None and tuple(up_add.shape) != (N, H // 2, W // 2, Co):
-        raise _lib.RcmvsError(f"conv1x1: up_add {tuple(up_add.shape)} does not match half of the output")
+    if up_add is not None and tuple(up_add.shape) != (N, (H + 1) // 2, (W + 1) // 2, Co):
+        raise _lib.RcmvsError(f"conv1x1: up_add {tuple(up_add.shape)} does not match half of the output (rounded up for an odd map)")
     y = torch.empty((N, H, W, Co), device=x.device, dtype=torch.float32)
     _lib.call("rcmvs_conv1x1_mfma_fwd" if mfma else "rcmvs_conv1x1_fwd", _chk(x, "x"), _chk(w_packed.blob, "w"), _opt(scale, "scale"), _opt(shift, "shift"),
               _opt(up_add, "up_add"), _chk(y, "y"), _opt(ysq_absmax, "ysq_absmax"), N, H, W, Ci, Co, int(relu), _stream())
@@ -484,23 +493,37 @@
 DEPTH_HEAD_IMPL = 0
 
 
-def depth_head(x8, w_prob_packed, planes, want_prob=False, x_absmax=None):
+def _next_planes(next_stage, B, h, w, device):
+    depth_values, (H, W), scale, ndepth, ratio = next_stage
+    if depth_values.shape[0] != B:
+        raise _lib.RcmvsError(f"next_stage: depth_values {tuple(depth_values.shape)} is not (B = {B}, ND)")
+    table = torch.empty((B, H // scale, W // scale, 2), device=device, dtype=torch.float32)
+    return table, (_chk(depth_values, "depth_values"), _chk(table, "next_planes"), H, W, int(scale), int(ndepth), ctypes.c_float(ratio), depth_values.shape[1])
+
+
+def depth_head(x8, w_prob_packed, planes, want_prob=False, x_absmax=None, next_stage=None):
     B, D, h, w, C = x8.shape
     if C != 8:
         raise _lib.RcmvsError("depth_head: the prob conv takes 8 channels")
     if x_absmax is not None and w_prob_packed.images != IMG_ALL:
         raise _lib.RcmvsError("depth_head: the fp16-pair form reads an image that a selectively packed weight does not hold")
+    if next_stage is not None and want_prob:
+        raise _lib.RcmvsError("depth_head: the launch that leaves the next stage's planes does not keep the probabilities")
     depth = torch.empty((B, h, w), device=x8.device, dtype=torch.float32)
     conf = torch.empty((B, h, w), device=x8.device, dtype=torch.float32)
-    one_launch = D == 8 and not (DEPTH_HEAD_IMPL & 1)
+    one_launch = D == 8 and not (DEPTH_HEAD_IMPL & 1) and next_stage is None
     prob = None if one_launch and not want_prob else torch.empty((B, D, h, w), device=x8.device, dtype=torch.float32)
-    _lib.call("rcmvs_depth_head_scaled_fwd", _chk(x8, "x8"), _opt(x_absmax, "x_absmax"), _chk(w_prob_packed.blob, "w_prob"), _chk(planes, "planes"),
-              _chk(depth, "depth"), _chk(conf, "conf"), _opt(prob, "prob"), B, D, h, w,
-              DEPTH_HEAD_IMPL | (0 if want_prob else 8), _stream())
+    args = (_chk(x8, "x8"), _opt(x_absmax, "x_absmax"), _chk(w_prob_packed.blob, "w_prob"), _chk(planes, "planes"),
+            _chk(depth, "depth"), _chk(conf, "conf"), _opt(prob, "prob"), B, D, h, w, DEPTH_HEAD_IMPL | (0 if want_prob else 8))
+    if next_stage is not None:
+        table, tail = _next_planes(next_stage, B, h, w, x8.device)
+        _lib.call("rcmvs_depth_head_planes_fwd", *args, *tail, _stream())
+        return depth, conf, table
+    _lib.call("rcmvs_depth_head_scaled_fwd", *args, _stream())
     return (depth, conf, prob) if want_prob else (depth, conf)
 
 
-def conv11_prob(t, t_absmax, w11_packed, scale, shift, res, res_absmax, coef, w_prob_packed, zchunk=0, planes=None):
+def conv11_prob(t, t_absmax, w11_packed, scale, shift, res, res_absmax, coef, w_prob_packed, zchunk=0, planes=None, next_stage=None):
     B, Dt, Ht, Wt, C = t.shape
     if C != 16 or tuple(res.shape) != (B, 2 * Dt, 2 * Ht, 2 * Wt, 8):
         raise _lib.RcmvsError(f"conv11_prob: t {tuple(t.shape)} / res {tuple(res.shape)} are not (B,Dt,Ht,Wt,16) / (B,2Dt,2Ht,2Wt,8)")
@@ -520,14 +543,21 @@
     if fused:
         return depth, conf
     if planes is not None:
-        return softmax_head(logits, planes)
+        return softmax_head(logits, planes, next_stage=next_stage)
     return logits
 
 
-def softmax_head(logits, planes, keep_prob=False):
+def softmax_head(logits, planes, keep_prob=False, next_stage=None):
     B, D, h, w = logits.shape
     depth = torch.empty((B, h, w), device=logits.device, dtype=torch.float32)
     conf = torch.empty((B, h, w), device=logits.device, dtype=torch.float32)
+    if next_stage is not None:
+        if keep_prob:
+            raise _lib.RcmvsError("softmax_head: the launch that leaves the next stage's planes does not keep the probabilities")
+        table, tail = _next_planes(next_stage, B, h, w, logits.device)
+        _lib.call("rcmvs_softmax_head_planes_fwd", _chk(logits, "logits"), _chk(planes, "planes"), _chk(depth, "depth"), _chk(conf, "conf"),
+                  B, D, h, w, *tail, _stream())
+        return depth, conf, table
     _lib.call("rcmvs_softmax_head_fwd", _chk(logits, "logits"), _chk(planes, "planes"), _chk(depth, "depth"), _chk(conf, "conf"),
               B, D, h, w, int(bool(keep_prob)), _stream())
     return depth, conf
```

Result: no change. 965.4 ref-scenes/s, median of 2 (-0.0%).
